# Azkellas/mesh_to_sdf

Measured on AMD Instinct MI355X. Metric: Mvoxels/s for generate_grid_sdf (512^3, 100k tris, Raycast), higher is better.
Workload: dtype f32; 1 GPU; generate_grid_sdf 512^3 grid, blob-100k (100000 tris, 50002 verts), SignMethod::Raycast, contiguous x-slabs over 1 GPU(s), whole grid resident on every GPU at the end of a step (delivery: single GPU, nothing to deliver), inputs/outputs resident in HBM; mesh=blob-100k, sign_method=Raycast, parallelism=xslab1, processes=1 (one per GPU), exchange=none, gather_chunks=1, piece_streams=1

## Files before the change

### mesh_to_sdf_amd/csrc/capi.hip

```cpp
#include <chrono>
#include <cmath>
#include <cstdarg>
#include <cstdio>
#include <cstdlib>
#include <algorithm>
#include <cstring>
#include <map>
#include <memory>
#include <mutex>
#include <thread>
#include <vector>

#include "../../include/m2s.h"
#include "capi_internal.h"
#include "common.h"
#include "sample.hip.h"
#include "tuning.h"

namespace m2s {

static thread_local char g_err[512] = "";

void set_error(const char* fmt, ...) {
  va_list ap;
// ... 2227 lines not shown
  M2S_HIP_CHECK(hipEventRecord(st->ev[2], c.stream));
  st->planes_done = nullptr;
  st->have_raw_seeds = false;
  if ((rc = remark_leaves(m, c, m->dm.leaf_max))) return rc;
  const NodeMom* moms = nullptr;
  if ((rc = mesh_winding_moments(m, c, *st, &moms))) return rc;
  if ((rc = run_grid_winding(ws, c, *st, m->dm, moms, g, slab_cells, o, d_err))) return rc;
  if (!c.sync) return park_async_events(m, *st, slab_cells, o.sdf ? 2 : 1);
  return finish_winding(c, *st, d_err, m->n_tris, slab_cells, o);
}

int m2s_cast_rays(const float* vertices, size_t n_vertices, const void* indices, size_t n_indices, int index_bytes, int topology,
                  const float* origins, const float* directions, size_t n_rays, const m2s_ray_opts* ropts, float* t_out, uint32_t* triangle_out,
                  float* uv_out, uint32_t* count_out, uint8_t* occluded_out, const m2s_opts* opts) {
  g_err[0] = 0;
  RayArgs o{t_out, triangle_out, uv_out, count_out, occluded_out, 0.0f, __builtin_inff()};
  int rc = check_mesh_args(vertices, n_vertices, indices, n_indices, index_bytes, topology);
  if (rc) return rc;
  if ((rc = check_ray_args(ropts, origins, directions, n_rays, opts, &o))) return rc;
  const size_t n_tris = m2s_triangle_count(n_vertices, n_indices, indices != nullptr, topology);
  if (!opts || opts->mem_kind == M2S_MEM_HOST) {
    if ((rc = check_host_indices(indices, n_indices, index_bytes, topology, n_vertices, n_tris))) return rc;
  }
  if (n_rays == 0) return M2S_OK;
  CallCtx c;
  DeviceState* st = nullptr;
  if ((rc = resolve_ctx(opts, &c, &st))) return rc;
  size_t need = (n_tris ? bvh_workspace_bytes(n_tris) : 0) + ray_workspace_bytes(c, n_rays) + 4096;
  if (c.mem_kind == M2S_MEM_HOST) need += align_up(n_vertices * 12) + align_up(n_indices * (size_t)(indices ? index_bytes : 0)) + 1024;
  if ((rc = ensure_capacity(*st, need))) return rc;
  Arena ws{st->base, st->cap, 0};
  int* d_err = ws.take<int>(16);
  M2S_HIP_CHECK(hipMemsetAsync(d_err, 0, 64, c.stream));
  M2S_HIP_CHECK(hipEventRecord(st->ev[0], c.stream));
  DeviceMesh mesh{};
  if (n_tris) {
    StagedMesh sm;
    if ((rc = stage_mesh(ws, c, vertices, n_vertices, indices, n_indices, index_bytes, &sm))) return rc;
    M2S_HIP_CHECK(hipEventRecord(st->ev[0], c.stream));
    rc = build_device_mesh(ws, c.stream, sm.d_verts, n_vertices, sm.d_indices, n_indices, index_bytes, topology, n_tris, d_err, &mesh,
                           nullptr, false, query_leaf_max(n_rays, n_tris, SIGN_NONE));
    if (rc) return rc;
  }
  M2S_HIP_CHECK(hipEventRecord(st->ev[1], c.stream));
  M2S_HIP_CHECK(hipEventRecord(st->ev[2], c.stream));
  st->planes_done = nullptr;
  if ((rc = run_cast_rays(ws, c, *st, mesh, origins, directions, n_rays, o))) return rc;
  return finish_call(c, *st, d_err, c.timings, n_tris, n_rays, false, true);
}

int m2s_mesh_cast_rays(m2s_mesh* m, const float* origins, const float* directions, size_t n_rays, const m2s_ray_opts* ropts, float* t_out,
                       uint32_t* triangle_out, float* uv_out, uint32_t* count_out, uint8_t* occluded_out, const m2s_opts* opts) {
  g_err[0] = 0;
  if (!m) return fail(M2S_ERR_BAD_ARG, "mesh is NULL");
  std::lock_guard<std::mutex> mlk(m->mu);
  RayArgs o{t_out, triangle_out, uv_out, count_out, occluded_out, 0.0f, __builtin_inff()};
  int rc = check_ray_args(ropts, origins, directions, n_rays, opts, &o);
  if (rc) return rc;
  m2s_opts mo;
  if ((rc = mesh_call_opts(m, opts, &mo))) return rc;
  if (n_rays == 0) return M2S_OK;
  CallCtx c;
  DeviceState* st = nullptr;
  if ((rc = resolve_ctx(&mo, &c, &st))) return rc;
  if ((rc = ensure_capacity(*st, ray_workspace_bytes(c, n_rays) + 8192))) return rc;
  Arena ws{st->base, st->cap, 0};
  int* d_err = ws.take<int>(16);
  if (c.sync) M2S_HIP_CHECK(hipMemsetAsync(d_err, 0, 64, c.stream));
  else d_err = m->d_err_async;
  if (!c.sync) reap_pending(m, false);
  M2S_HIP_CHECK(hipEventRecord(st->ev[0], c.stream));
  M2S_HIP_CHECK(hipEventRecord(st->ev[1], c.stream));
  M2S_HIP_CHECK(hipEventRecord(st->ev[2], c.stream));
  st->planes_done = nullptr;
  DeviceMesh none{};
  if (m->n_tris && (rc = remark_leaves(m, c, m->dm.leaf_max))) return rc;
  if ((rc = run_cast_rays(ws, c, *st, m->n_tris ? m->dm : none, origins, directions, n_rays, o))) return rc;
  if (!c.sync) return park_async_events(m, *st, n_rays, 1);
  return finish_call(c, *st, d_err, c.timings, m->n_tris, n_rays, false, true);
}

int m2s_sample_surface(const float* vertices, size_t n_vertices, const void* indices, size_t n_indices, int index_bytes, int topology,
                       size_t n_samples, const m2s_surface_sample_opts* sopts, float* point_out, uint32_t* triangle_out, float* uv_out,
                       float* normal_out, double* area_out, const m2s_opts* opts) {
  g_err[0] = 0;
  SampleArgs o{point_out, triangle_out, uv_out, normal_out, area_out, 0, 0};
  int rc = check_mesh_args(vertices, n_vertices, indices, n_indices, index_bytes, topology);
  if (rc) return rc;
  if ((rc = check_sample_args(sopts, n_samples, opts, &o))) return rc;
  const size_t n_tris = m2s_triangle_count(n_vertices, n_indices, indices != nullptr, topology);
  if (n_tris > ((size_t)1 << 25)) return fail(M2S_ERR_BAD_ARG, "more than 2^25 triangles");
  if (!opts || opts->mem_kind == M2S_MEM_HOST) {
    if ((rc = check_host_indices(indices, n_indices, index_bytes, topology, n_vertices, n_tris))) return rc;
  }
  if (n_tris == 0) return sample_of_nothing(o, n_samples);
  CallCtx c;
  DeviceState* st = nullptr;
  if ((rc = resolve_ctx(opts, &c, &st))) return rc;
  size_t need = sample_table_bytes(n_tris) + sample_scratch_bytes(n_tris) + sample_workspace_bytes(c, n_samples) + 4096;
  if (c.mem_kind == M2S_MEM_HOST) need += align_up(n_vertices * 12) + align_up(n_indices * (size_t)(indices ? index_bytes : 0)) + 1024;
  if ((rc = ensure_capacity(*st, need))) return rc;
  Arena ws{st->base, st->cap, 0};
  int* d_err = ws.take<int>(16);
  M2S_HIP_CHECK(hipMemsetAsync(d_err, 0, 64, c.stream));
  StagedMesh sm;
  if ((rc = stage_mesh(ws, c, vertices, n_vertices, indices, n_indices, index_bytes, &sm))) return rc;
  M2S_HIP_CHECK(hipEventRecord(st->ev[0], c.stream));
  M2S_HIP_CHECK(hipEventRecord(st->ev[1], c.stream));
  M2S_HIP_CHECK(hipEventRecord(st->ev[2], c.stream));
  st->planes_done = nullptr;
  SampleTable tb;
  if (sample_table_carve(ws, ws, n_tris, &tb)) return fail(M2S_ERR_HIP, "internal: workspace");
  const SampleSrc src{sm.d_verts, sm.d_indices, (uint32_t)n_vertices, index_bytes, topology, nullptr, nullptr, (uint32_t)n_tris};
  uint32_t amax_bits = 0;
  uint64_t W = 0;
  if ((rc = make_sample_table(c, *st, src, tb, d_err, &amax_bits, &W))) return rc;
  if (amax_bits == 0 || W == 0) return sample_of_nothing(o, n_samples);
  if (o.area) *o.area = sample_total_area(amax_bits, W);
  if ((rc = run_sample_surface(ws, c, *st, src, tb, W, n_samples, o))) return rc;
  return finish_call(c, *st, d_err, c.timings, n_tris, n_samples, false, true);
}

int m2s_mesh_sample_surface(m2s_mesh* m, size_t n_samples, const m2s_surface_sample_opts* sopts, float* point_out, uint32_t* triangle_out,
                            float* uv_out, float* normal_out, double* area_out, const m2s_opts* opts) {
  g_err[0] = 0;
  if (!m) return fail(M2S_ERR_BAD_ARG, "mesh is NULL");
  std::lock_guard<std::mutex> mlk(m->mu);
  SampleArgs o{point_out, triangle_out, uv_out, normal_out, area_out, 0, 0};
  int rc = check_sample_args(sopts, n_samples, opts, &o);
  if (rc) return rc;
  m2s_opts mo;
  if ((rc = mesh_call_opts(m, opts, &mo))) return rc;
  if (m->n_tris == 0) return sample_of_nothing(o, n_samples);
  CallCtx c;
  DeviceState* st = nullptr;
  if ((rc = resolve_ctx(&mo, &c, &st))) return rc;
  if ((rc = ensure_capacity(*st, (m->samp_mem ? 0 : sample_scratch_bytes(m->n_tris)) + sample_workspace_bytes(c, n_samples) + 8192))) return rc;
  Arena ws{st->base, st->cap, 0};
  int* d_err = ws.take<int>(16);
  if (c.sync) M2S_HIP_CHECK(hipMemsetAsync(d_err, 0, 64, c.stream));
  else d_err = m->d_err_async;
  if (!c.sync) reap_pending(m, false);
  M2S_HIP_CHECK(hipEventRecord(st->ev[0], c.stream));
  M2S_HIP_CHECK(hipEventRecord(st->ev[1], c.stream));
  M2S_HIP_CHECK(hipEventRecord(st->ev[2], c.stream));
  st->planes_done = nullptr;
  if ((rc = remark_leaves(m, c, m->dm.leaf_max))) return rc;
  const SampleSrc src{nullptr, nullptr, 0, 4, M2S_TRIANGLE_LIST, m->dm.corners, m->dm.slot_of, (uint32_t)m->n_tris};
  if (!m->samp_mem) {
    char* block = nullptr;
    const size_t bytes = sample_table_bytes(m->n_tris);
    M2S_HIP_CHECK(hipMalloc((void**)&block, bytes));
    Arena table{block, bytes, 0};
    SampleTable tb;
    rc = sample_table_carve(table, ws, m->n_tris, &tb) ? fail(M2S_ERR_HIP, "internal: workspace") : 0;
    if (!rc) rc = make_sample_table(c, *st, src, tb, nullptr, &m->samp_amax_bits, &m->samp_W);
    if (rc) { (void)hipFree(block); return rc; }
    m->samp_mem = block;
    m->samp = tb;
    m->samp.A = nullptr;
    m->samp.tile_sum = nullptr;
  }
  if (m->samp_amax_bits == 0 || m->samp_W == 0) return sample_of_nothing(o, n_samples);
  if (o.area) *o.area = sample_total_area(m->samp_amax_bits, m->samp_W);
  if ((rc = run_sample_surface(ws, c, *st, src, m->samp, m->samp_W, n_samples, o))) return rc;
  if (!c.sync) return park_async_events(m, *st, n_samples, 1);
  return finish_call(c, *st, d_err, c.timings, m->n_tris, n_samples, false, true);
}

int m2s_peer_bandwidth(const float* src, float* const* peers, uint32_t n_peers, size_t n_cells, int device, float* gbps_each, float* gbps_all) {
  g_err[0] = 0;
  if (!src || (n_peers && !peers) || n_peers > M2S_MAX_PEERS) return fail(M2S_ERR_BAD_ARG, "m2s_peer_bandwidth: bad arguments");
  if (n_cells == 0 || n_peers == 0) { if (gbps_all) *gbps_all = 0.0f; return M2S_OK; }
  int ndev = 0;
  if (hipGetDeviceCount(&ndev) != hipSuccess || ndev <= 0) return fail(M2S_ERR_HIP, "no HIP device available");
  if (device < 0) M2S_HIP_CHECK(hipGetDevice(&device));
  if (device >= ndev) return fail(M2S_ERR_BAD_ARG, "device %d out of range (%d devices)", device, ndev);
  int prev_device = device;
  (void)hipGetDevice(&prev_device);
  struct Guard {
    hipStream_t st = nullptr;
    hipEvent_t a = nullptr, b = nullptr;
    int restore;
    ~Guard() {
      if (a) (void)hipEventDestroy(a);
      if (b) (void)hipEventDestroy(b);
      if (st) (void)hipStreamDestroy(st);
      (void)hipSetDevice(restore);
    }
  } guard;
  guard.restore = prev_device;
  M2S_HIP_CHECK(hipSetDevice(device));
  M2S_HIP_CHECK(hipStreamCreateWithFlags(&guard.st, hipStreamNonBlocking));
  M2S_HIP_CHECK(hipEventCreate(&guard.a));
  M2S_HIP_CHECK(hipEventCreate(&guard.b));
  const hipStream_t st = guard.st;
  const hipEvent_t a = guard.a, b = guard.b;
  int rc = M2S_OK;
  auto timed = [&](const PeerOut& po, float* gbps) -> int {
    float best = 0.0f;
    for (int rep = 0; rep < 4; ++rep) {
      M2S_HIP_CHECK(hipEventRecord(a, st));
      const int r = launch_push_cells(st, src, po, 0, n_cells);
      if (r) return r;
      M2S_HIP_CHECK(hipEventRecord(b, st));
      M2S_HIP_CHECK(hipStreamSynchronize(st));
      float ms = 0.0f;
      M2S_HIP_CHECK(hipEventElapsedTime(&ms, a, b));
      if (rep && ms > 0.0f) best = std::max(best, (float)((double)n_cells * 4.0 * po.n / (ms * 1e-3) / 1e9));
    }
    *gbps = best;
    return 0;
  };
  for (uint32_t k = 0; k < n_peers && !rc; ++k) {
    if (!peers[k]) { rc = fail(M2S_ERR_BAD_ARG, "m2s_peer_bandwidth: peers[%u] is NULL", k); break; }
    PeerOut one{};
    one.n = 1;
    one.p[0] = peers[k];
    float g = 0.0f;
    rc = timed(one, &g);
    if (gbps_each) gbps_each[k] = g;
  }
  if (!rc && gbps_all) {
    PeerOut all{};
    all.n = n_peers;
    for (uint32_t k = 0; k < n_peers; ++k) all.p[k] = peers[k];
    rc = timed(all, gbps_all);
  }
  return rc;
}

int m2s_tuning_set(const char* name, const char* value) {
  clear_error();
  if (tuning_set(name, value) != 0) return fail(M2S_ERR_BAD_ARG, "m2s_tuning_set: unknown knob or unparsable value: %s=%s", name ? name : "(null)", value ? value : "(default)");
  return M2S_OK;
}
int m2s_tuning_describe(char* buffer, int capacity) { return tuning_describe(buffer, capacity); }

int m2s_debug_mesh_digest(m2s_mesh* m, uint64_t out[8]) {
  g_err[0] = 0;
  if (!m || !out) return fail(M2S_ERR_BAD_ARG, "NULL argument");
  std::lock_guard<std::mutex> mlk(m->mu);
  M2S_HIP_CHECK(hipSetDevice(m->device));
  M2S_HIP_CHECK(hipDeviceSynchronize());
  const size_t n = m->n_tris, nn = n ? 2 * n - 1 : 0;
  const void* ptr[7] = {m->dm.tris, m->dm.planes, m->dm.nodes, m->dm.ext, m->dm.cen, m->dm.slot_of, m->dm.scene};
  const size_t bytes[7] = {n * sizeof(TriRec), n * sizeof(TriPlanes), nn * sizeof(NodeRec), nn * sizeof(NodeExt), n * 16, n * 4, n ? 32u : 0u};
  std::vector<unsigned char> h;
  for (int k = 0; k < 7; ++k) {
    uint64_t f = 1469598103934665603ull;
    if (bytes[k]) {
      h.resize(bytes[k]);
      M2S_HIP_CHECK(hipMemcpy(h.data(), ptr[k], bytes[k], hipMemcpyDeviceToHost));
      for (size_t i = 0; i < bytes[k]; ++i) { f ^= h[i]; f *= 1099511628211ull; }
    }
    out[k] = f;
  }
  out[7] = n;
  return M2S_OK;
}

int m2s_debug_cut_code(uint32_t n_nodes, uint32_t start, uint32_t len, uint32_t out[3]) {
  g_err[0] = 0;
  if (!out || n_nodes == 0 || n_nodes > (1u << 26) || len == 0 || start >= n_nodes || len > n_nodes - start) return fail(M2S_ERR_BAD_ARG, "bad range");
  cut_word_roundtrip(n_nodes, start, len, &out[0], &out[1], &out[2]);
  return M2S_OK;
}

int m2s_debug_leaf_sizes(const m2s_grid* grid, size_t n_tris, size_t n_queries, uint32_t out[3]) {
  g_err[0] = 0;
  if (!grid || !out) return fail(M2S_ERR_BAD_ARG, "NULL argument");
  GridParams g;
  size_t slab_cells = 0;
  const int rc = fill_grid_params(grid, nullptr, &g, &slab_cells);
  if (rc) return rc;
  out[0] = grid_leaf_max(g, n_tris);
  out[1] = query_leaf_max(n_queries, n_tris, SIGN_RAYS3);
  out[2] = query_walk_is_lane(n_queries, n_tris, SIGN_RAYS3) ? 1u : 0u;
  return M2S_OK;
}

int m2s_debug_grid_walk_choice_slab(const m2s_grid* grid, const m2s_opts* opts, size_t n_tris, size_t n_nodes, uint32_t leaf_max, int algorithm, uint32_t out[8]) {
  g_err[0] = 0;
  if (!grid || !out) return fail(M2S_ERR_BAD_ARG, "NULL argument");
  GridParams g;
  size_t slab_cells = 0;
  const int rc = fill_grid_params(grid, opts, &g, &slab_cells);
  if (rc) return rc;
  const GridWalkChoice ch = choose_grid_walk(g, n_tris, n_nodes, leaf_max, false, algorithm, tuning());
  out[0] = (uint32_t)ch.path;
  out[1] = ch.seeds ? 1u : 0u;
  out[2] = (uint32_t)ch.cut_levels;
  out[3] = ch.group_waves;
  out[4] = ch.split ? 1u : 0u;
  out[5] = ch.split_forced ? 1u : 0u;
  out[6] = (uint32_t)ch.defer;
  out[7] = choose_grid_walk_for_sizing(g, n_tris).split ? 1u : 0u;
  return M2S_OK;
}
int m2s_debug_grid_walk_choice(const m2s_grid* grid, size_t n_tris, size_t n_nodes, uint32_t leaf_max, int algorithm, uint32_t out[8]) {
  return m2s_debug_grid_walk_choice_slab(grid, nullptr, n_tris, n_nodes, leaf_max, algorithm, out);
}

}
```

### mesh_to_sdf_amd/csrc/common.h

```cpp
#pragma once
#include <functional>
#include <hip/hip_runtime.h>
#include <stddef.h>
#include <stdint.h>

namespace m2s {

struct alignas(32) TriRec {
  float ax, ay, az;
  uint32_t cls;
  float bx, by, bz;
  uint32_t index;
  float cx, cy, cz;
  float pad0;
  float abx, aby, abz, nrx;
  float acx, acy, acz, nry;
  float bcx, bcy, bcz, nrz;
};
static_assert(sizeof(TriRec) == 96, "TriRec must be 96 bytes");

struct alignas(32) NodeRec {
  float mnx, mny, mnz;
  uint32_t skip;
  float mxx, mxy, mxz;
  int32_t tri;
};
static_assert(sizeof(NodeRec) == 32, "NodeRec must be 32 bytes");

struct alignas(16) NodeExt {
  float cx, cy, cz, R;
  float nx, ny, nz, mid;
  float half;
  uint32_t skip;
  int32_t tri;
  uint32_t pad;
};
constexpr uint32_t EXT_TRIVIAL_ABOVE = 2048;
static_assert(sizeof(NodeExt) == 48, "NodeExt must be 48 bytes");

struct alignas(64) TriPlanes {
  float nx, ny, nz, dn;
  float m0x, m0y, m0z, o0;
  float m1x, m1y, m1z, o1;
  float m2x, m2y, m2z, o2;
};
static_assert(sizeof(TriPlanes) == 64, "TriPlanes must be 64 bytes");

struct DeviceMesh {
  const TriRec* tris;
  const float4* corners;
  const TriPlanes* planes;
  const float4* cen;
  const float4* cen_raw;
  const uint32_t* slot_of;
  const NodeRec* nodes;
  const NodeExt* ext;
  unsigned long long* stats;
  uint32_t n_tris;
  uint32_t n_nodes;
  uint32_t leaf_max;
  const uint32_t* slot_first;
  const int* scene;
};

__device__ __forceinline__ float mesh_scale(const DeviceMesh& m) { return __int_as_float(m.scene[6]); }

struct GridParams {
  float first[3];
  float size[3];
  uint32_t n[3];
  uint32_t xb, xe;
  uint32_t nzw;
  uint64_t out_off;
  uint32_t bl[3];
  uint32_t sz_magic, sy_magic;
  uint32_t xl_cap;
  uint32_t chunk_log, period;
};
__host__ __device__ __forceinline__ uint32_t slab_x(const GridParams& g, uint32_t v) {
  return g.xb + (v >> g.chunk_log) * g.period + (v & ((1u << g.chunk_log) - 1u));
}

inline void set_super_brick_magic(GridParams& g) {
  const uint64_t nbx = (g.n[0] + (1u << g.bl[0]) - 1u) >> g.bl[0], nby = (g.n[1] + (1u << g.bl[1]) - 1u) >> g.bl[1],
                 nbz = (g.n[2] + (1u << g.bl[2]) - 1u) >> g.bl[2];
  const uint64_t sy = (nby + 7) >> 3, sz = (nbz + 7) >> 3, n_max = (nbx + 1) * sy * sz;
  const uint64_t d_max = sy > sz ? sy : sz;
  const bool safe = n_max * d_max < (1ull << 32);
  g.sz_magic = (safe && sz > 1) ? (uint32_t)(((1ull << 32) + sz - 1) / sz) : 0u;
  g.sy_magic = (safe && sy > 1) ? (uint32_t)(((1ull << 32) + sy - 1) / sy) : 0u;
}

inline void choose_brick_shape(const float size[3], uint32_t bl[3]) {
  bl[0] = bl[1] = bl[2] = 2;
  float s[3];
  for (int k = 0; k < 3; ++k) {
    s[k] = size[k] < 0 ? -size[k] : size[k];
    if (!(s[k] > 0.0f) || !(s[k] < 3.0e38f)) return;
  }
  float best = -1.0f;
  for (uint32_t a = 0; a <= 6; ++a)
    for (uint32_t b = 0; a + b <= 6; ++b) {
      const uint32_t c = 6 - a - b;
      const float e[3] = {s[0] * (float)(1u << a), s[1] * (float)(1u << b), s[2] * (float)(1u << c)};
      const float mx = e[0] > e[1] ? (e[0] > e[2] ? e[0] : e[2]) : (e[1] > e[2] ? e[1] : e[2]);
      const float mn = e[0] < e[1] ? (e[0] < e[2] ? e[0] : e[2]) : (e[1] < e[2] ? e[1] : e[2]);
      const float ratio = mx / mn;
      const bool cube = a == 2 && b == 2;
      if (best < 0.0f || ratio < best * 0.999f || (cube && ratio <= best * 1.001f)) { best = ratio; bl[0] = a; bl[1] = b; bl[2] = c; }
    }
}

constexpr uint32_t MAX_PEERS = 15;
struct PeerOut {
  float* p[MAX_PEERS];
  uint32_t n;
  uint32_t unit_log;
  uint32_t rows;
  uint32_t units;
  uint32_t* progress;
};

enum : int { ERRF_INDEX_OOB = 1, ERRF_NAN = 2, ERRF_TRAIL_TIMEOUT = 4, ERRF_BUILD_TIMEOUT = 8, ERRF_SPLIT_OVERFLOW = 16 };

enum : int {
  MODE_UNSIGNED = 0,
  MODE_NORMAL_FOLD = 1,
  MODE_NEAREST_NORMAL = 2
};
enum : int {
  SIGN_NONE = 0,
  SIGN_GRID_PLANE = 1,
  SIGN_RAYS3 = 2,
  SIGN_XRAY_ALL = 3
};

#define M2S_HIP_CHECK(expr)                                                   \
  do {                                                                        \
    hipError_t _e = (expr);                                                   \
    if (_e != hipSuccess) {                                                   \
      ::m2s::set_error("%s failed: %s (%s:%d)", #expr, hipGetErrorString(_e), __FILE__, __LINE__); \
      return M2S_ERR_HIP_INTERNAL;                                            \
    }                                                                         \
  } while (0)

constexpr int M2S_ERR_HIP_INTERNAL = -4;
void set_error(const char* fmt, ...);

struct Arena {
  char* base = nullptr;
  size_t cap = 0;
  size_t off = 0;
  template <class T>
  T* take(size_t count, size_t align = 256) {
    size_t o = (off + align - 1) / align * align;
    size_t bytes = count * sizeof(T);
    if (o + bytes > cap) return nullptr;
    off = o + bytes;
    return reinterpret_cast<T*>(base + o);
  }
};

hipError_t sort_pairs_u64(void* tmp, size_t& bytes, const uint64_t* keys_in, uint64_t* keys_out, const uint32_t* vals_in, uint32_t* vals_out, size_t n,
                          unsigned begin_bit, unsigned end_bit, hipStream_t st);
hipError_t sort_pairs_u32(void* tmp, size_t& bytes, const uint32_t* keys_in, uint32_t* keys_out, const uint32_t* vals_in, uint32_t* vals_out, size_t n,
                          unsigned begin_bit, unsigned end_bit, hipStream_t st);
hipError_t select_flagged_indices(void* tmp, size_t& bytes, const uint8_t* flags, uint32_t* out, uint32_t* count, size_t n, hipStream_t st);
void warm_bvh(hipStream_t st);
void warm_sign(hipStream_t st);
void warm_distance(hipStream_t st);
void warm_seeds(hipStream_t st);
void warm_cut(hipStream_t st);
void warm_brute(hipStream_t st);
void warm_query_order(hipStream_t st);
void warm_peer_push(hipStream_t st);
void warm_serde(hipStream_t st);
void warm_client(hipStream_t st);
void warm_sortlib(hipStream_t st);
void warm_sortlib_query(hipStream_t st);
void warm_grid_query(hipStream_t st);
void warm_rays(hipStream_t st);
void warm_sample(hipStream_t st);
size_t bvh_workspace_bytes(size_t n_tris);
int build_device_mesh(Arena& ws, hipStream_t st, const float* d_verts, size_t n_verts, const void* d_indices,
                      size_t n_indices, int index_bytes, int topology, size_t n_tris, int* d_err, DeviceMesh* out,
                      const std::function<int(const float4*, const TriRec*, int)>* after_setup = nullptr, bool records_only = false,
                      uint32_t leaf_max = 2, uint64_t job_cells = ~0ull);
bool query_walk_is_lane(size_t n_q, size_t n_tris, int sign_src);
uint32_t query_leaf_max(size_t n_q, size_t n_tris, int sign_src);
uint32_t grid_leaf_max(const GridParams& g, size_t n_tris);
int set_leaf_size(hipStream_t st, DeviceMesh* mesh, uint32_t leaf_max);

size_t sign_workspace_bytes(const GridParams& g, size_t n_tris);
int build_grid_sign_plane(Arena& ws, hipStream_t st, const DeviceMesh& mesh, const GridParams& g,
                          const uint32_t** d_inside_plane, bool slab_only);

size_t grid_distance_workspace_bytes(const GridParams& g, size_t n_tris);
constexpr uint32_t SPLIT_MAX_ROUNDS = 6, SPLIT_CNT_WORDS = 16 + 16 * (SPLIT_MAX_ROUNDS + 1);
struct SplitCtl {
  uint32_t* cnt = nullptr;
  uint32_t* slot_packet = nullptr;
  uint32_t* acc = nullptr;
  uint4* items = nullptr;
  uint32_t cap_slots = 0, cap_items = 0;
  uint32_t grace = 0;
  uint32_t patience_q8 = 0;
  uint32_t idle_below = 0;
  uint32_t emit_min = 0, emit_max = 0;
  uint32_t rounds = 3;
};
struct Tuning;
struct GridWalkChoice {
  enum Path { NOTHING, ALL_PAIRS_SPLIT , ALL_PAIRS , LANE, GROUP, PACKET };
  Path path = NOTHING;
  bool seeds = false;
  int cut_levels = 0;
  uint32_t group_waves = 0;
  bool split = false;
  bool split_forced = false;
  int defer = 0;
};
GridWalkChoice choose_grid_walk(const GridParams& g, size_t n_tris, size_t n_nodes, uint32_t leaf_max, bool counting, int algorithm, const Tuning& tn);
GridWalkChoice choose_grid_walk_for_sizing(const GridParams& g, size_t n_tris);
struct GridWalkPlan {
  GridWalkChoice choice;
  const uint32_t* seeds = nullptr;
  uint32_t seed_shift = 0, seed_ny = 0, seed_nz = 0;
  const uint32_t* cut_lists = nullptr;
  uint32_t cut_log = 0, cut_ny = 0, cut_nz = 0;
  SplitCtl split;
  const uint2* group_top = nullptr;
  uint32_t* brute_acc = nullptr;
};
bool grid_is_tiny(const GridParams& g, size_t n_tris, int algorithm, bool raycast);
bool grid_is_tiny(const GridParams& g, size_t n_tris, int algorithm, bool raycast, const Tuning& tn);
struct SeedLattice {
  uint32_t* ids = nullptr;
  uint32_t ny = 0, nz = 0;
  size_t points = 0;
  uint32_t shift = 0;
};
bool grid_walk_wants_seeds(const GridParams& g, size_t n_tris, int algorithm);
uint32_t host_packet_bricks(const GridParams& g);
int launch_grid_seeds(Arena& ws, hipStream_t st, const float4* cen, uint32_t n_tris, const GridParams& g, SeedLattice* out);
void launch_seed_remap(hipStream_t st, uint32_t* ids, size_t n, const uint32_t* slot_of, uint32_t n_tris);
void launch_grid_cut(hipStream_t st, const DeviceMesh& mesh, const GridParams& g, const uint32_t* seeds, uint32_t seed_shift, uint32_t seed_ny,
                     uint32_t seed_nz, uint32_t* lists, uint32_t* coarse);
void launch_query_cut(hipStream_t st, const DeviceMesh& mesh, const uint32_t* seeds, uint32_t launched, uint32_t* lists, const float4* centres,
                      const uint32_t* table, const GridParams* d_lat);
int launch_grid_brute_split(hipStream_t st, const DeviceMesh& mesh, const GridParams& g, int mode, const uint32_t* plane, uint32_t* acc, uint32_t real,
                            float* d_out, int* d_err, const PeerOut& peers);
int launch_grid_brute(hipStream_t st, const DeviceMesh& mesh, const GridParams& g, int mode, const uint32_t* plane, float* d_out, int* d_err,
                      uint32_t packets, const PeerOut& peers);
int launch_query_brute(hipStream_t st, const DeviceMesh& mesh, const float* d_queries, uint32_t n_q, int mode, int sign_src, float* d_out, int* d_err);
int prepare_grid_walk(Arena& ws, hipStream_t st, const DeviceMesh& mesh, const GridParams& g, int algorithm, bool pipelined,
                      GridWalkPlan* plan, const SeedLattice* raw_seeds = nullptr);
int launch_grid_walk(hipStream_t st, const DeviceMesh& mesh, const GridParams& g, int mode, const uint32_t* d_inside_plane,
                     const GridWalkPlan& plan, uint32_t bx_off, float* d_out, int* d_err, const PeerOut* peers = nullptr);
int launch_push_cells(hipStream_t st, const float* src, const PeerOut& peers, uint64_t first, uint64_t count);
uint32_t trail_unit_log(const GridParams& g);
uint32_t trail_units(const GridParams& g);
uint32_t trail_rows(const GridParams& g);
int launch_push_trailing(hipStream_t st, const float* src, const PeerOut& peers, const GridParams& g, int* d_err);
int launch_grid_distance(Arena& ws, hipStream_t st, const DeviceMesh& mesh, const GridParams& g, int mode,
                         const uint32_t* d_inside_plane, int algorithm, float* d_out, int* d_err,
                         hipEvent_t ev_before_final, hipEvent_t wait_before_final = nullptr, bool pipelined = false,
                         const SeedLattice* raw_seeds = nullptr, hipEvent_t wait_raw_seeds = nullptr,
                         const PeerOut* peers = nullptr);
void cut_word_roundtrip(uint32_t n_nodes, uint32_t start, uint32_t len, uint32_t* word, uint32_t* first, uint32_t* end);
size_t query_workspace_bytes(size_t n_q);
bool query_is_tiny(size_t n_q, size_t n_tris, int algorithm, int sign_src);
int launch_query_brute_split(Arena& ws, hipStream_t st, const DeviceMesh& mesh, const float* d_queries, size_t n_q, int mode, int sign_src,
                             float* d_out, int* d_err);
struct QueryPlan {
  size_t n_q = 0;
  const int* qb = nullptr;
  const uint32_t* perm = nullptr;
  const float4* sorted = nullptr;
  const uint32_t* table = nullptr;
  const float4* centres = nullptr;
  const GridParams* lat = nullptr;
  uint32_t launched = 0;
  bool lane_walk = false, seeds = false;
};
struct QuerySeeds {
  uint32_t* ids = nullptr;
  bool raw = false;
};
int prepare_query_walk(Arena& ws, hipStream_t st, const float* d_queries, size_t n_q, size_t n_tris, int sign_src, int algorithm, QueryPlan* plan,
                       hipEvent_t after_lattice = nullptr);
int launch_query_seeds(Arena& ws, hipStream_t st, const float4* cen, uint32_t n_tris, const QueryPlan& plan, bool raw, QuerySeeds* out);
int launch_query_walk(Arena& ws, hipStream_t st, const DeviceMesh& mesh, const float* d_queries, const QueryPlan& plan,
                      int mode, int sign_src, int algorithm, float* d_out, int* d_err, const QuerySeeds* pre = nullptr);
int launch_query_distance(Arena& ws, hipStream_t st, const DeviceMesh& mesh, const float* d_queries, size_t n_q,
                          int mode, int sign_src, int algorithm, float* d_out, int* d_err);

struct ClosestOut {
  uint32_t* tri;
  float* point;
  float* dist;
  uint64_t off;
};
int launch_closest_grid(hipStream_t st, const DeviceMesh& mesh, const GridParams& g, const float* d_dist, uint64_t dist_off, int algorithm,
                        const ClosestOut& out);
int launch_closest_queries(hipStream_t st, const DeviceMesh& mesh, const float* d_queries, const uint32_t* perm, size_t n_q, const float* d_dist,
                           int algorithm, const ClosestOut& out);

struct alignas(64) NodeMom {
  float cx, cy, cz;
  float r;
  float ax, ay, az;
  float m[9];
};
static_assert(sizeof(NodeMom) == 64, "NodeMom must be 64 bytes");
struct WindingOut {
  float* w;
  float* sdf;
  uint64_t off;
};
int launch_winding_moments(hipStream_t st, const DeviceMesh& mesh, NodeMom* moms);
int launch_winding_grid(hipStream_t st, const DeviceMesh& mesh, const NodeMom* moms, const GridParams& g, float beta, float threshold,
                        const float* d_dist, uint64_t dist_off, int algorithm, const WindingOut& out);
int launch_winding_queries(hipStream_t st, const DeviceMesh& mesh, const NodeMom* moms, const float* d_queries, const uint32_t* perm, size_t n_q,
                           float beta, float threshold, const float* d_dist, int algorithm, const WindingOut& out);


struct RayOut {
  float* t;
  uint32_t* tri;
  float* uv;
  uint32_t* count;
  uint8_t* occluded;
};
int launch_cast_rays(hipStream_t st, const DeviceMesh& mesh, const float* d_org, const float* d_dir, size_t n_rays, float t_min, float t_max,
                     int algorithm, const RayOut& out);

struct SampleSrc {
  const float* verts;
  const void* indices;
  uint32_t n_verts;
  int index_bytes, topology;
  const float4* corners;
  const uint32_t* slot_of;
  uint32_t n_tris;
};
constexpr uint32_t SAMPLE_TOP = 2048;
struct SampleTable {
  uint64_t* C;
  uint64_t* top;
  uint32_t* hdr;
  float* A;
  uint64_t* tile_sum;
};
struct SampleOut {
  float* point;
  uint32_t* tri;
  float* uv;
  float* normal;
};
size_t sample_table_bytes(size_t n_tris);
size_t sample_scratch_bytes(size_t n_tris);
int sample_table_carve(Arena& table, Arena& scratch, size_t n_tris, SampleTable* tb);
int launch_sample_table(hipStream_t st, const SampleSrc& src, const SampleTable& tb, int* d_err);
int launch_sample_surface(hipStream_t st, const SampleSrc& src, const SampleTable& tb, uint64_t W, uint64_t seed, uint64_t first, size_t n_samples,
                          int algorithm, const SampleOut& out);

struct GridQuery {
  float start[3], end[3], cs[3];
  int64_t n[3];
  uint64_t nyz;
  float iso, outside;
  float eps;
  uint32_t max_steps;
};
int launch_sample_grid(hipStream_t st, const GridQuery& q, int mode, const float* d, const float* pts, uint64_t n, float* value_out,
                       float* normal_out);
int launch_raymarch_grid(hipStream_t st, const GridQuery& q, int mode, const float* d, const float* org, const float* dir, uint64_t n,
                         float* hit_out, uint32_t* steps_out, float* normal_out);


struct wire_bytes { uint8_t b[120]; uint32_t n; };
int launch_write_bytes(hipStream_t st, uint8_t* d_dst, const uint8_t* bytes, uint32_t n);
int launch_encode_f32(hipStream_t st, const float* d_values, uint64_t n, uint8_t* d_dst);
int launch_encode_points(hipStream_t st, const float* d_points, uint64_t n, uint8_t* d_dst);
int launch_decode_f32(hipStream_t st, const uint8_t* d_src, uint64_t n, float* d_out, int* d_err);
int launch_decode_points(hipStream_t st, const uint8_t* d_src, uint64_t n, float* d_out, int* d_err);

size_t order_workspace_bytes(size_t n);
int launch_order_cells(Arena& ws, hipStream_t st, const float* d_dist, size_t n, uint32_t* d_ordered, float* d_limits);
struct InstanceDev {
  const void* vertices;
  const uint32_t* indices;
  uint64_t stride;
  float m[16];
};
size_t merge_workspace_bytes();
int launch_merge_instances(Arena& ws, hipStream_t st, const InstanceDev* d_inst, const uint64_t* d_vfirst, const uint64_t* d_ifirst,
                           uint32_t n_inst, uint64_t n_vertices, uint64_t n_indices, float* d_vertices, uint32_t* d_indices,
                           float* d_bbox);

}
```

### mesh_to_sdf_amd/csrc/dist.hip.h

```cpp
#pragma once
#include "common.h"
#include "walk.hip.h"

namespace m2s {

namespace {

#ifndef M2S_CUT_MAX
#define M2S_CUT_MAX 15
#endif
__host__ __device__ __forceinline__ uint32_t cut_start_bits(uint32_t n_nodes) {
  uint32_t b = 1;
  while (b < 27u && (1u << b) < n_nodes) ++b;
  return b;
}
__host__ __device__ __forceinline__ uint32_t cut_decode_len(uint32_t code, uint32_t M) { return (code & ((1u << M) - 1u)) << (code >> M); }
__host__ __device__ __forceinline__ uint32_t cut_encode_len(uint32_t len, uint32_t M) {
  if (len < (1u << M)) return len;
  uint32_t e = (32u - (uint32_t)__builtin_clz(len)) - M;
  uint32_t mant = (len + (1u << e) - 1u) >> e;
  if (mant == (1u << M)) { mant >>= 1; ++e; }
  return (e << M) | mant;
}
constexpr uint32_t CUT_MAX = M2S_CUT_MAX, CUT_WORDS = M2S_CUT_MAX + 1;
static_assert(M2S_CUT_MAX <= 15, "the range count has four bits");
struct CutList {
  const uint32_t* lists;
  uint32_t log, ny, nz;
  uint32_t bx_off;
  const float4* centres;
};
constexpr uint32_t CUTC_S_LOG = 3, CUTC_S = 1u << CUTC_S_LOG, CUTC_WORDS = 8, CUTC_MAX = CUTC_WORDS - 1;
static_assert(CUTC_S * CUTC_WORDS == 64, "a fine wave fetches its block's coarse record with one load, lane = word");

__device__ __forceinline__ bool query_packet_range(const uint32_t* __restrict__ table, uint32_t packet, uint32_t n_q,
                                                   uint32_t* first, uint32_t* cnt) {
  uint32_t f = packet * 64u, c = 64u;
  if (table != nullptr) {
    const uint32_t count = table[0];
    if (packet >= count) return false;
    if (table[1] == 0u) {
      f = table[2u + packet];
      c = (packet + 1u < count ? table[3u + packet] : n_q) - f;
    }
  }
  if (f >= n_q) return false;
  *first = f;
  *cnt = min(c, n_q - f);
  return true;
}
__device__ __forceinline__ uint32_t query_lattice_cell(const GridParams& L, float x, float y, float z) {
  const float q0[3] = {x, y, z};
  uint32_t cell[3];
  for (int k = 0; k < 3; ++k) {
    float f = (q0[k] - L.first[k]) / L.size[k] + 0.5f;
    f = (f == f) ? fminf(fmaxf(f, 0.0f), (float)(L.n[k] - 1)) : 0.0f;
    cell[k] = min((uint32_t)f, L.n[k] - 1);
  }
  return (cell[0] * L.n[1] + cell[1]) * L.n[2] + cell[2];
}
constexpr uint32_t QL = 64;

template <int M, int S>
struct WalkForm { static constexpr int MODE = M, SIGN = S; };
template <class F>
void for_grid_form(int mode, bool planes, F&& f) {
  if (mode == MODE_UNSIGNED && planes) f(WalkForm<MODE_UNSIGNED, SIGN_GRID_PLANE>{});
  else if (mode == MODE_UNSIGNED) f(WalkForm<MODE_UNSIGNED, SIGN_NONE>{});
  else f(WalkForm<MODE_NORMAL_FOLD, SIGN_NONE>{});
}
template <class F>
void for_query_form(int mode, int sign_src, F&& f) {
  if (mode == MODE_UNSIGNED && sign_src == SIGN_RAYS3) f(WalkForm<MODE_UNSIGNED, SIGN_RAYS3>{});
  else if (mode == MODE_UNSIGNED) f(WalkForm<MODE_UNSIGNED, SIGN_NONE>{});
  else if (mode == MODE_NORMAL_FOLD) f(WalkForm<MODE_NORMAL_FOLD, SIGN_NONE>{});
  else f(WalkForm<MODE_NEAREST_NORMAL, SIGN_NONE>{});
}

struct BrickCounts { uint32_t nb[3]; uint64_t real, grid; uint32_t padded; };
static bool slab_is_empty(const GridParams& g) { return g.xe <= g.xb || g.n[1] == 0 || g.n[2] == 0; }
BrickCounts brick_counts(const GridParams& g) {
  BrickCounts c;
  c.nb[0] = bricks_along(g.xe - g.xb, g.bl[0]), c.nb[1] = bricks_along(g.n[1], g.bl[1]), c.nb[2] = bricks_along(g.n[2], g.bl[2]);
  c.real = (uint64_t)c.nb[0] * c.nb[1] * c.nb[2];
  c.grid = (uint64_t)bricks_along(g.n[0], g.bl[0]) * c.nb[1] * c.nb[2];
  const uint32_t xl = super_brick_xlog(c.nb[0], g.xl_cap);
  c.padded = ((c.nb[0] + (1u << xl) - 1u) >> xl) * ((c.nb[1] + 7) >> 3) * ((c.nb[2] + 7) >> 3) * (64u << xl);
  return c;
}
static size_t cut_blocks(const GridParams& g, uint32_t log) {
  const BrickCounts bc = brick_counts(g);
  return (size_t)bricks_along(bc.nb[0], log) * bricks_along(bc.nb[1], log) * bricks_along(bc.nb[2], log);
}

}

}
```

### mesh_to_sdf_amd/csrc/distance.hip

```cpp
#include <algorithm>
#include <cmath>
#include <cstdio>
#include <cstdlib>
#include <cstring>
#include <type_traits>

#include "common.h"
#include "geo.hip.h"
#include "tuning.h"
#include "walk.hip.h"
#include "dist.hip.h"

namespace m2s {

namespace {

template <int AXIS>
__device__ __forceinline__ uint32_t stab_count(const DeviceMesh& mesh, f3 p) {
  uint32_t count = 0;
  uint32_t node = 0;
  while (node < mesh.n_nodes) {
    node = __builtin_amdgcn_readfirstlane(node);
    const NodeRec nr = record_at(mesh.nodes, node);
    const bool hit = ray_meets_box<AXIS>(p, mk3(nr.mnx, nr.mny, nr.mnz), mk3(nr.mxx, nr.mxy, nr.mxz));
// ... 91 lines not shown
__device__ __forceinline__ uint32_t split_peek(const uint32_t* addr) {
  uint32_t v;
  const uint32_t zero = 0;
  asm volatile("s_nop 4\n\tglobal_load_dword %0, %1, %2 nt\n\ts_waitcnt vmcnt(0)" : "=v"(v) : "v"(zero), "s"(addr));
  return (uint32_t)__builtin_amdgcn_readfirstlane((int)v);
}
__device__ __forceinline__ void split_poke(uint32_t* addr, uint32_t value) {
  const uint32_t zero = 0;
  asm volatile("s_nop 4\n\tglobal_store_dword %0, %1, %2" : : "v"(zero), "v"(value), "s"(addr));
}
__device__ __forceinline__ uint32_t split_now() { return (uint32_t)__builtin_amdgcn_s_memrealtime(); }
__device__ __forceinline__ void split_arm(SplitState& sp, const SplitCtl& ctl, uint32_t round, bool may_suspend) {
  if (ctl.cnt == nullptr || !may_suspend) return;
  sp.flag_addr = split_flag_addr(ctl, round);
  sp.next_check = ctl.grace;
  sp.grace = ctl.grace;
  sp.patience_q8 = ctl.patience_q8;
}
__device__ __forceinline__ bool split_stragglers_only(const SplitState& sp) {
  const uint32_t up = split_peek(sp.flag_addr);
  if (up == 0u) return false;
  const uint32_t start = split_peek(sp.flag_addr + 8), now = split_now();
  const uint32_t fill = up - start;
  const uint32_t allowed = (uint32_t)(((unsigned long long)fill * sp.patience_q8) >> 8);
  return now - up >= allowed;
}

template <int MODE>
__device__ __forceinline__ bool split_handover(const SplitCtl& split, uint32_t packet, uint32_t range, uint32_t off, const Best<MODE>& best, int* err) {
  const uint32_t lane = threadIdx.x & 63u;
  uint32_t slot = 0, idx = 0;
  if (lane == 0u) slot = atomicAdd(&split.cnt[0], 1u);
  slot = __builtin_amdgcn_readfirstlane(slot);
  if (slot >= split.cap_slots) return false;
  if (lane == 0u) idx = atomicAdd(&split.cnt[2], 1u);
  idx = __builtin_amdgcn_readfirstlane(idx);
  if (idx >= split.cap_items) {
    if (lane == 0u) split.slot_packet[slot] = 0xffffffffu;
    return false;
  }
  constexpr uint32_t AW = MODE == MODE_NORMAL_FOLD ? 128u : 64u;
  uint32_t* acc = split.acc + (size_t)slot * AW;
  acc[lane] = __float_as_uint(best.d2);
  if (MODE == MODE_NORMAL_FOLD) {
    acc[64 + lane] = __float_as_uint(best.d2pos);
    if (best.nan) atomicOr(err, ERRF_NAN);
  }
  if (lane == 0u) {
    split.items[idx] = make_uint4(packet, off, range, slot | SPLIT_CONTINUATION);
    split.slot_packet[slot] = packet;
  }
  return true;
}

struct EmitState {
  uint4* list = nullptr;
  uint32_t* count = nullptr;
  uint32_t cap = 0;
  uint32_t base = 0, used = 0, room = 0;
  uint32_t min_bytes = 0xffffffffu, max_bytes = 0;
  uint32_t packet = 0, slot = 0;
};
__device__ __forceinline__ void emit_begin(EmitState& em, const SplitCtl& ctl, uint32_t next_round, uint32_t packet, uint32_t slot) {
  em.list = ctl.items + (size_t)(next_round - 1u) * ctl.cap_items;
  em.count = ctl.cnt + 1u + next_round;
  em.cap = ctl.cap_items;
  em.min_bytes = ctl.emit_min;
  em.max_bytes = ctl.emit_max;
  em.packet = packet;
  em.slot = slot;
}
__device__ __forceinline__ void emit_close(EmitState& em) {
  const uint32_t i = em.base + em.used + (threadIdx.x & 63u);
  if (i < em.base + em.room && i < em.cap) em.list[i] = make_uint4(em.packet, 0u, 0u, em.slot);
  em.used = em.room;
}
__device__ __forceinline__ void emit_reserve(EmitState& em) {
  uint32_t base = 0;
  if ((threadIdx.x & 63u) == 0u) base = atomicAdd(em.count, 64u);
  em.base = __builtin_amdgcn_readfirstlane(base);
  em.used = 0;
  em.room = 64u;
  if (em.base + 64u > em.cap) {
    emit_close(em);
    em.room = 0;
    em.min_bytes = 0xffffffffu;
  }
}

template <int MODE>
struct DeferLayout {
  static constexpr uint32_t SLOT_WORDS = MODE == MODE_NORMAL_FOLD ? 192u : MODE == MODE_NEAREST_NORMAL ? 128u : 64u;
  static constexpr uint32_t DWORDS = (256u + SLOT_WORDS) / 2u;
};
constexpr uint32_t DEFER_DIRECT_LANES = 48;
struct DeferQueue {
  uint32_t* q;
  uint32_t* slot;
  uint32_t head, n;
  uint32_t* q1;
  uint32_t head1, n1;
};
__device__ __forceinline__ void wave_lds_sync() {
  __builtin_amdgcn_fence(__ATOMIC_RELEASE, "wavefront");
  __builtin_amdgcn_wave_barrier();
  __builtin_amdgcn_fence(__ATOMIC_ACQUIRE, "wavefront");
}
template <int MODE>
__device__ __forceinline__ unsigned long long defer_key(const Best<MODE>& x) {
  return ((unsigned long long)__float_as_uint(x.d2) << 32) | ((unsigned long long)(x.idx & 0x7fffffffu) << 1) | (x.pos ? 0ull : 1ull);
}
template <int MODE>
__device__ __forceinline__ DeferQueue defer_begin(unsigned long long* lds) {
  const uint32_t lane = threadIdx.x & 63u;
  DeferQueue dq = {reinterpret_cast<uint32_t*>(lds), reinterpret_cast<uint32_t*>(lds) + 256, 0u, 0u, reinterpret_cast<uint32_t*>(lds) + 128, 0u, 0u};
  if (MODE == MODE_NEAREST_NORMAL) reinterpret_cast<unsigned long long*>(dq.slot)[lane] = 0x7f800000ffffffffull;
  else {
    dq.slot[lane] = 0x7f800000u;
    if (MODE == MODE_NORMAL_FOLD) { dq.slot[64u + lane] = 0x7f800000u; dq.slot[128u + lane] = 0u; }
  }
  return dq;
}
template <int MODE>
__device__ __forceinline__ void defer_flush(const DeviceMesh& mesh, f3 p, DeferQueue& dq, Best<MODE>& best) {
  const uint32_t lane = threadIdx.x & 63u;
  wave_lds_sync();
  const uint32_t take = min(dq.n, 64u);
  const bool valid = lane < take;
  const uint32_t e = valid ? dq.q[(dq.head + lane) & 127u] : 0u;
  const uint32_t v = e & 63u, t = e >> 6;
  const f3 pv = mk3(__shfl(p.x, (int)v), __shfl(p.y, (int)v), __shfl(p.z, (int)v));
  Best<MODE> one;
  eval_triangle<MODE>(one, pv, mesh.tris[t]);
  if (valid) {
    if (MODE == MODE_NEAREST_NORMAL) atomicMin(&reinterpret_cast<unsigned long long*>(dq.slot)[v], defer_key<MODE>(one));
    else {
      atomicMin(&dq.slot[v], __float_as_uint(one.d2));
      if (MODE == MODE_NORMAL_FOLD) {
        atomicMin(&dq.slot[64u + v], __float_as_uint(one.d2pos));
        if (one.nan) dq.slot[128u + v] = 1u;
      }
    }
  }
  dq.head = (dq.head + take) & 127u;
  dq.n -= take;
  wave_lds_sync();
  if (MODE == MODE_NEAREST_NORMAL) {
    const unsigned long long kk = reinterpret_cast<const unsigned long long*>(dq.slot)[lane];
    if (kk < defer_key<MODE>(best)) { best.d2 = __uint_as_float((uint32_t)(kk >> 32)); best.idx = (uint32_t)(kk >> 1) & 0x7fffffffu; best.pos = (kk & 1ull) == 0ull; }
  } else {
    best.d2 = fminf(best.d2, __uint_as_float(dq.slot[lane]));
    if (MODE == MODE_NORMAL_FOLD) { best.d2pos = fminf(best.d2pos, __uint_as_float(dq.slot[64u + lane])); best.nan |= dq.slot[128u + lane] != 0u; }
  }
}
template <int MODE>
__device__ __forceinline__ bool defer_pretest(const DeviceMesh& mesh, f3 p, float thr, DeferQueue& dq, Best<MODE>& best) {
  const uint32_t lane = threadIdx.x & 63u;
  wave_lds_sync();
  const uint32_t take = min(dq.n1, 64u);
  const bool valid = lane < take;
  const uint32_t e = valid ? dq.q1[(dq.head1 + lane) & 127u] : 0u;
  const uint32_t v = e & 63u, t = e >> 6;
  const f3 pv = mk3(__shfl(p.x, (int)v), __shfl(p.y, (int)v), __shfl(p.z, (int)v));
  const float tv = __shfl(thr, (int)v);
  const bool pass = valid & !(planes_dist2(pv, mesh.planes[t]) > tv);
  dq.head1 = (dq.head1 + take) & 127u;
  dq.n1 -= take;
  const unsigned long long rb = __ballot(pass);
  if (rb == 0ull) return false;
  const uint32_t rank = __builtin_amdgcn_mbcnt_hi((uint32_t)(rb >> 32), __builtin_amdgcn_mbcnt_lo((uint32_t)rb, 0u));
  if (pass) dq.q[(dq.head + dq.n + rank) & 127u] = e;
  dq.n += (uint32_t)__popcll(rb);
  if (dq.n < 64u) return false;
  defer_flush<MODE>(mesh, p, dq, best);
  return true;
}
template <int MODE>
__device__ __forceinline__ void defer_drain(const DeviceMesh& mesh, f3 p, float slack, DeferQueue& dq, Best<MODE>& best) {
  while (dq.n1 != 0u) defer_pretest<MODE>(mesh, p, prune_bound(best.d2, slack), dq, best);
  while (dq.n != 0u) defer_flush<MODE>(mesh, p, dq, best);
}

template <int MODE, bool STATS, bool BUDGET, bool EMIT = false, bool HANDOVER = false, int DEFER = 0>
__device__ __forceinline__ void walk_span(const DeviceMesh& mesh, f3 p, float slack, Best<MODE>& best, float& thr, uint32_t& off,
                                          uint32_t end, WalkStats& st, SplitState& sp, EmitState* emp = nullptr, DeferQueue* dqp = nullptr) {
  constexpr uint32_t NB = (uint32_t)sizeof(NodeExt);
  while (off < end) {
    off = __builtin_amdgcn_readfirstlane(off);
    const NodeExt nr = record_at_bytes<NodeExt>(mesh.ext, off);
    if (STATS) ++st.box;
    const float ed2 = ext_dist2(p, nr);
    if (STATS) st.node_lanes += (uint32_t)__popcll(__ballot(!(ed2 > thr)));
    if (STATS && __ballot(!(ed2 > thr)) == 0ull) {
      ++st.pruned;
      const float vx = p.x - nr.cx, vy = p.y - nr.cy, vz = p.z - nr.cz;
      const float t = nr.nz * vz + nr.ny * vy + nr.nx * vx, sl = fmaxf(fabsf(t - nr.mid) - nr.half, 0.0f);
      if (__ballot(!(sl * sl > thr)) == 0ull) ++st.slab;
      const float rs = __builtin_amdgcn_sqrtf(nr.R * nr.R + (fabsf(nr.mid) + nr.half) * (fabsf(nr.mid) + nr.half));
      const float sq = fmaxf(__builtin_amdgcn_sqrtf(vx * vx + vy * vy + vz * vz) - rs, 0.0f);
      if (__ballot(!(sq * sq > thr)) == 0ull) ++st.sphere;
    }
    if (__ballot(!(ed2 > thr)) == 0ull) { off = nr.skip; continue; }
    if (nr.tri >= 0) {
      const uint32_t cnt = (nr.skip - off + NB) / (2u * NB);
      if (DEFER == 3) {
        DeferQueue& dq = *dqp;
        const bool want = !(ed2 > thr);
        const unsigned long long wb = __ballot(want);
        const uint32_t rank = __builtin_amdgcn_mbcnt_hi((uint32_t)(wb >> 32), __builtin_amdgcn_mbcnt_lo((uint32_t)wb, 0u));
        const uint32_t wn = (uint32_t)__popcll(wb);
        for (uint32_t k = 0; k < cnt; ++k) {
          if (want) dq.q1[(dq.head1 + dq.n1 + rank) & 127u] = (threadIdx.x & 63u) | (((uint32_t)nr.tri + k) << 6);
          dq.n1 += wn;
          if (dq.n1 >= 64u) {
            if (BUDGET) sp.units += 4u;
            if (defer_pretest<MODE>(mesh, p, thr, dq, best)) thr = prune_bound(best.d2, slack);
          }
        }
      } else
      for (uint32_t k = 0; k < cnt; ++k) {
        if (STATS) { ++st.ext; st.pre_lanes += (uint32_t)__popcll(__ballot(!(ed2 > thr))); }
        const TriPlanes tp = record_at(mesh.planes, (uint32_t)nr.tri + k);
        const bool reach = !(planes_dist2(p, tp) > thr);
        const unsigned long long rb = __ballot(reach);
        if (rb != 0ull) {
          if (STATS) { ++st.leaf; st.pairs += (uint32_t)__popcll(rb); }
          if (DEFER != 0 && !(DEFER == 2 && (uint32_t)__popcll(rb) >= DEFER_DIRECT_LANES)) {
            DeferQueue& dq = *dqp;
            const uint32_t rank = __builtin_amdgcn_mbcnt_hi((uint32_t)(rb >> 32), __builtin_amdgcn_mbcnt_lo((uint32_t)rb, 0u));
            if (reach) dq.q[(dq.head + dq.n + rank) & 127u] = (threadIdx.x & 63u) | (((uint32_t)nr.tri + k) << 6);
            dq.n += (uint32_t)__popcll(rb);
            if (dq.n >= 64u) {
              if (BUDGET) sp.units += 4u;
              defer_flush<MODE>(mesh, p, dq, best);
              thr = prune_bound(best.d2, slack);
            }
          } else {
            if (BUDGET) sp.units += 4u;
            const TriRec tr = record_at_vec(mesh.tris, (uint32_t)nr.tri + k);
            eval_triangle_leaf<MODE>(best, p, tr, reach);
            thr = prune_bound(best.d2, slack);
          }
        }
      }
      off = nr.skip;
      if (BUDGET) {
        sp.units += 3u + cnt;
        if (sp.units >= sp.next_check) {
          bool go;
          if (HANDOVER) go = split_stragglers_only(sp);
          else {
            go = sp.flag_seen;
            if (!go && split_peek(sp.flag_addr) != 0u) { sp.flag_seen = true; sp.next_check = sp.units + sp.grace; }
          }
          if (go) {
            if (off < end || HANDOVER) { sp.suspended = true; sp.resume_end = end; end = off; if (HANDOVER) *sp.n_ranges = 0u; }
            sp.next_check = 0xffffffffu;
          } else if (HANDOVER || !sp.flag_seen) {
            sp.next_check = sp.units + SPLIT_CHECK_EVERY;
          }
        }
      }
    } else {
      if (EMIT) {
        EmitState& em = *emp;
        const uint32_t bytes = nr.skip - off;
        if (bytes >= em.min_bytes && bytes <= em.max_bytes) {
          if (em.used == em.room) emit_reserve(em);
          if (em.used < em.room) {
            if ((threadIdx.x & 63u) == 0u) em.list[em.base + em.used] = make_uint4(em.packet, off, nr.skip, em.slot);
            ++em.used;
            off = nr.skip;
            continue;
          }
        }
      }
      off = off + NB;
    }
  }
}

__device__ __forceinline__ void store_grid_result(float* __restrict__ out, size_t out_index, float result, bool store, const GridParams& g,
                                                  const GridBrick& vox, const PeerOut& peers, int lane) {
  if (peers.progress != nullptr) {
    if (store) __hip_atomic_store(&out[out_index], result, __ATOMIC_RELAXED, __HIP_MEMORY_SCOPE_AGENT);
    asm volatile("s_waitcnt vmcnt(0)" ::: "memory");
    if (lane == 0) {
      const uint32_t unit = vox.bx >> peers.unit_log;
      const uint32_t nbx = bricks_along(g.xe - g.xb, g.bl[0]), nbz = bricks_along(g.n[2], g.bl[2]);
      const uint32_t bricks = min((unit + 1u) << peers.unit_log, nbx) - (unit << peers.unit_log);
      const uint32_t old = __hip_atomic_fetch_add(&peers.progress[peers.units + unit * peers.rows + vox.by], 1u, __ATOMIC_RELAXED, __HIP_MEMORY_SCOPE_AGENT);
      if (old + 1u == bricks * nbz) __hip_atomic_fetch_add(&peers.progress[unit], 1u, __ATOMIC_RELAXED, __HIP_MEMORY_SCOPE_AGENT);
    }
    return;
  }
  if (store) out[out_index] = result;
  if (peers.n != 0u && store) {
    const size_t gi = out_index + (size_t)g.out_off;
    for (uint32_t i = 0; i < peers.n; ++i) peers.p[i][gi] = result;
  }
}

template <bool GRID, int MODE, int SIGN, bool STATS, bool SPLIT, int DEFER = 0>
__global__ __launch_bounds__(64) __attribute__((amdgpu_waves_per_eu(8, 8))) void k_packet(DeviceMesh mesh, GridParams g, const float4* __restrict__ qsorted,
                                               const uint32_t* __restrict__ perm, uint32_t n_q,
                                               const uint32_t* __restrict__ plane, float* __restrict__ out,
                                               int* __restrict__ err, uint32_t n_packets,
                                               const uint32_t* __restrict__ seed_in, uint32_t seed_shift,
                                               uint32_t seed_ny, uint32_t seed_nz,
                                               const GridParams* __restrict__ seed_lattice, CutList cut, PeerOut peers, SplitCtl split) {
  const int lane = threadIdx.x & 63;
  if (SPLIT && (blockIdx.x < 8u || blockIdx.x + 8u >= gridDim.x) && lane == 0) {
    const uint32_t t = split.idle_below  ? 0u : split_now();
    if (blockIdx.x < 8u) split_poke(split_flag_addr(split, 0u) + 8, t);
    if (blockIdx.x + 8u >= gridDim.x) split_poke(split_flag_addr(split, 0u), t | 1u);
  }
  const uint32_t block = xcd_remap(blockIdx.x);
  const uint32_t packet = (uint32_t)__builtin_amdgcn_readfirstlane((int)block);
  if (packet >= n_packets) return;

  f3 p;
  size_t out_index;
  bool store;
  GridBrick vox{};
  if (GRID) {
    vox = grid_lane_voxel(g, packet, lane);
    if (!vox.brick_in_grid) return;
    p = grid_point(g, vox);
    out_index = ((size_t)vox.x * g.n[1] + vox.y) * g.n[2] + vox.z - (size_t)g.out_off;
    store = vox.in_range;
  } else {
    uint32_t first, cnt;
    if (!query_packet_range(plane, packet, n_q, &first, &cnt)) return;
    const uint32_t i = first + min((uint32_t)lane, cnt - 1u);
    const float4 q = qsorted[i];
    p = mk3(q.x, q.y, q.z);
    out_index = perm[i];
    store = (uint32_t)lane < cnt;
  }

  Best<MODE> best;
  WalkStats st;
  uint32_t st_ranges = 0, st_band = 0, st_rbytes = 0;
  if (mesh.n_nodes) {
    const float scale = fmaxf(mesh_scale(mesh), fmaxf(fabsf(p.x), fmaxf(fabsf(p.y), fabsf(p.z))));
    const float slack = 4.0e-6f * scale + (MODE == MODE_NORMAL_FOLD ? 2.5e-6f : 0.0f);
    SplitState sp;
    if (SPLIT) split_arm(sp, split, 0u, true);
    __shared__ unsigned long long defer_lds[DEFER ? DeferLayout<MODE>::DWORDS : 1];
    DeferQueue dq = {nullptr, nullptr, 0u, 0u};
    if (DEFER) dq = defer_begin<MODE>(defer_lds);

    constexpr uint32_t NB = (uint32_t)sizeof(NodeExt);
    const uint32_t* cl = nullptr;
    uint32_t n_ranges = 1, cut_off_v = 0, cut_end_v = (lane == 1) ? mesh.n_nodes * NB : 0u;
    if (SPLIT) sp.n_ranges = &n_ranges;
    if (cut.lists != nullptr) {
      const uint32_t cb = GRID ? __builtin_amdgcn_readfirstlane((((vox.bx + cut.bx_off) >> cut.log) * cut.ny + (vox.by >> cut.log)) * cut.nz + (vox.bz >> cut.log))
                               : packet;
      cl = cut.lists + (size_t)cb * CUT_WORDS;
      const uint32_t cw = cl[(uint32_t)lane & 15u];
      const uint32_t cS = cut_start_bits(mesh.n_nodes), cfirst = cw & ((1u << cS) - 1u);
      const uint32_t clen = ((cw >> cS) & ((1u << (27u - cS)) - 1u)) << (cw >> 27);
      cut_off_v = cfirst * NB;
      cut_end_v = min(cfirst + clen, mesh.n_nodes) * NB;
      n_ranges = __builtin_amdgcn_readfirstlane(cw);
    }
    if (seed_in != nullptr) {
      uint32_t sidx = packet;
      if (GRID) {
        sidx = (((vox.bx + cut.bx_off) >> seed_shift) * seed_ny + (vox.by >> seed_shift)) * seed_nz + (vox.bz >> seed_shift);
      } else {
        const GridParams L = *seed_lattice;
        float q0[3] = {__shfl(p.x, 0), __shfl(p.y, 0), __shfl(p.z, 0)};
        if (cut.centres != nullptr) {
          const float4 c = cut.centres[packet];
          q0[0] = c.x; q0[1] = c.y; q0[2] = c.z;
        }
        sidx = __builtin_amdgcn_readfirstlane(query_lattice_cell(L, q0[0], q0[1], q0[2]));
      }
      const uint32_t slot = __builtin_amdgcn_readfirstlane(min(seed_in[sidx], mesh.n_tris - 1));
      const TriRec tr = record_at(mesh.tris, slot);
      eval_triangle<MODE>(best, p, tr);
    } else {
      const f3 c = {__shfl(p.x, 0), __shfl(p.y, 0), __shfl(p.z, 0)};
      uint32_t n = 0;
      NodeRec nr = mesh.nodes[0];
      while (nr.tri < 0) {
        const uint32_t l = n + 1;
        const NodeRec nl = mesh.nodes[l];
        const uint32_t r = nl.skip;
        const NodeRec nrr = mesh.nodes[r];
        const float dl = box_dist2(c, nl.mnx, nl.mny, nl.mnz, nl.mxx, nl.mxy, nl.mxz);
        const float dr = box_dist2(c, nrr.mnx, nrr.mny, nrr.mnz, nrr.mxx, nrr.mxy, nrr.mxz);
        const bool go_left = __builtin_amdgcn_readfirstlane((int)(dl <= dr)) != 0;
        n = go_left ? l : r;
        nr = go_left ? nl : nrr;
      }
      const TriRec tr = mesh.tris[nr.tri];
      eval_triangle<MODE>(best, p, tr);
    }

    float thr = prune_bound(best.d2, slack);
    if (STATS && GRID) {
      const float cells = __shfl(__builtin_amdgcn_sqrtf(best.d2), 0) / fabsf(g.size[0]);
      st_band = cells < 1.0f ? 0u : min(7u, 1u + (uint32_t)__builtin_amdgcn_readfirstlane((int)floorf(log2f(cells))));
      st_band = __builtin_amdgcn_readfirstlane(st_band);
    }
    const int passes = (STATS && mesh.stats != nullptr && mesh.stats[7] == 2ull) ? 2 : 1;
    for (int pass = 0; pass < passes; ++pass) {
      if (pass == 1) { st.box = 0; st.ext = 0; st.leaf = 0; }
      if (STATS) st_ranges = n_ranges;
      uint32_t range = 0, off = 0;
      for (; range < n_ranges; ++range) {
        off = (uint32_t)__builtin_amdgcn_readlane((int)cut_off_v, (int)(1u + range));
        const uint32_t end = (uint32_t)__builtin_amdgcn_readlane((int)cut_end_v, (int)(1u + range));
        if (STATS) st_rbytes += end - off;
        walk_span<MODE, STATS, SPLIT, false, SPLIT, DEFER>(mesh, p, slack, best, thr, off, end, st, sp, nullptr, &dq);
      }
      if (DEFER) defer_drain<MODE>(mesh, p, slack, dq, best);
      if (SPLIT && sp.suspended) {
        if (!split_handover<MODE>(split, packet, range - 1u, off, best, err)) atomicOr(err, ERRF_SPLIT_OVERFLOW);
        return;
      }
    }
  }

  if (STATS && mesh.stats != nullptr && lane == 0) {
    atomicAdd(&mesh.stats[0], (unsigned long long)st.box);
    atomicAdd(&mesh.stats[1], (unsigned long long)st.ext);
    atomicAdd(&mesh.stats[2], (unsigned long long)st.leaf);
    atomicAdd(&mesh.stats[3], 1ull);
    atomicAdd(&mesh.stats[4], (unsigned long long)st.pruned);
    atomicAdd(&mesh.stats[5], (unsigned long long)st.slab);
    atomicAdd(&mesh.stats[6], (unsigned long long)st.sphere);
    atomicMax(&mesh.stats[72], (unsigned long long)st.box);
    atomicMax(&mesh.stats[73], (unsigned long long)st.leaf);
    atomicMax(&mesh.stats[74], (unsigned long long)(st.box + st.ext + 4u * st.leaf));
    atomicAdd(&mesh.stats[75], (unsigned long long)st.node_lanes);
    atomicAdd(&mesh.stats[76], (unsigned long long)st.pre_lanes);
    atomicAdd(&mesh.stats[77], (unsigned long long)st.pairs);
    unsigned long long* q = mesh.stats + 8 + 8 * st_band;
    atomicAdd(&q[0], (unsigned long long)st.box);
    atomicAdd(&q[1], (unsigned long long)st.ext);
    atomicAdd(&q[2], (unsigned long long)st.leaf);
    atomicAdd(&q[3], 1ull);
    atomicAdd(&q[4], (unsigned long long)st_ranges);
    atomicAdd(&q[5], (unsigned long long)st.pairs);
    atomicAdd(&q[6], (unsigned long long)st_rbytes);
    atomicAdd(&q[7], (unsigned long long)(st_rbytes <= 4096u ? 1u : 0u));
    const uint32_t units = st.box + st.ext + 4u * st.leaf;
    atomicAdd(&mesh.stats[80 + (31 - __builtin_clz(units | 1u))], 1ull);
  }

  bool negate = false;
  if (MODE == MODE_UNSIGNED) {
    if (SIGN == SIGN_GRID_PLANE) {
      const size_t w = ((size_t)vox.x * g.n[1] + vox.y) * g.nzw + (vox.z >> 5);
      negate = (plane[w] >> (vox.z & 31u)) & 1u;
    } else if (SIGN == SIGN_RAYS3) {
      __shared__ uint32_t ray_lds[DEFER != 0 ? 192 : 1];
      const uint32_t cx = DEFER != 0 ? stab_count_dense<0>(mesh, p, ray_lds) : stab_count<0>(mesh, p);
      const uint32_t cy = DEFER != 0 ? stab_count_dense<1>(mesh, p, ray_lds) : stab_count<1>(mesh, p);
      uint32_t cz = cx;
      if (__ballot(((cx ^ cy) & 1u) != 0u) != 0ull) cz = DEFER != 0 ? stab_count_dense<2>(mesh, p, ray_lds) : stab_count<2>(mesh, p);
      negate = ((cx & 1u) + (cy & 1u) + (cz & 1u)) > 1u;
    }
  }
  if (MODE == MODE_NORMAL_FOLD && best.nan) atomicOr(err, ERRF_NAN);
  const float result = finish<MODE>(best, negate);
  if (GRID) store_grid_result(out, out_index, result, store, g, vox, peers, lane);
  else if (store) out[out_index] = result;
}

constexpr uint32_t GROUP_MAX_WAVES = 4, TOP_LOG = 8, TOP_SUBTREES = 1u << TOP_LOG;
__global__ __launch_bounds__(TOP_SUBTREES) void k_tree_top(DeviceMesh mesh, uint2* __restrict__ top) {
  constexpr uint32_t NB = (uint32_t)sizeof(NodeExt);
  const uint32_t sub = threadIdx.x;
  uint32_t off = 0, end = mesh.n_nodes * NB;
  for (uint32_t lv = 0; lv < TOP_LOG && off < end; ++lv) {
    const NodeExt* nr = reinterpret_cast<const NodeExt*>(reinterpret_cast<const char*>(mesh.ext) + off);
    const uint32_t rest = sub & ((1u << (TOP_LOG - lv)) - 1u);
    if (nr->tri >= 0) { if (rest != 0u) end = off; break; }
    const uint32_t skip = nr->skip, left = off + NB;
    const uint32_t right = reinterpret_cast<const NodeExt*>(reinterpret_cast<const char*>(mesh.ext) + left)->skip;
    if ((sub >> (TOP_LOG - 1u - lv)) & 1u) { off = right; end = skip; } else { off = left; end = right; }
  }
  top[sub] = make_uint2(off, end);
}
template <int MODE, int SIGN>
__global__ __launch_bounds__(64 * GROUP_MAX_WAVES) __attribute__((amdgpu_waves_per_eu(8, 8))) void k_packet_group(
    DeviceMesh mesh, GridParams g, const uint32_t* __restrict__ plane, float* __restrict__ out, int* __restrict__ err, uint32_t n_packets,
    const uint32_t* __restrict__ seed_in, uint32_t seed_shift, uint32_t seed_ny, uint32_t seed_nz, uint32_t bx_off, const uint2* __restrict__ top, PeerOut peers) {
  static_assert(MODE == MODE_UNSIGNED || MODE == MODE_NORMAL_FOLD, "grid modes");
  const int lane = threadIdx.x & 63;
  const uint32_t wave = (uint32_t)__builtin_amdgcn_readfirstlane((int)(threadIdx.x >> 6));
  const uint32_t packet = (uint32_t)__builtin_amdgcn_readfirstlane((int)xcd_remap(blockIdx.x));
  if (packet >= n_packets) return;
  const GridBrick vox = grid_lane_voxel(g, packet, lane);
  if (!vox.brick_in_grid) return;
  const f3 p = grid_point(g, vox);
  const size_t out_index = ((size_t)vox.x * g.n[1] + vox.y) * g.n[2] + vox.z - (size_t)g.out_off;

  extern __shared__ unsigned long long group_lds[];
  const uint32_t GROUP_WAVES = blockDim.x >> 6;
  uint32_t* const lds = reinterpret_cast<uint32_t*>(group_lds);
  DeferQueue dq = {lds + wave * 256u, lds + GROUP_WAVES * 256u, 0u, 0u, lds + wave * 256u + 128u, 0u, 0u};
  if (wave == 0u) {
    dq.slot[lane] = 0x7f800000u;
    if (MODE == MODE_NORMAL_FOLD) { dq.slot[64 + lane] = 0x7f800000u; dq.slot[128 + lane] = 0u; }
  }
  Best<MODE> best;
  if (mesh.n_nodes) {
    const float scale = fmaxf(mesh_scale(mesh), fmaxf(fabsf(p.x), fmaxf(fabsf(p.y), fabsf(p.z))));
    const float slack = 4.0e-6f * scale + (MODE == MODE_NORMAL_FOLD ? 2.5e-6f : 0.0f);
    uint32_t slot = 0;
    if (seed_in != nullptr) {
      const uint32_t sidx = (((vox.bx + bx_off) >> seed_shift) * seed_ny + (vox.by >> seed_shift)) * seed_nz + (vox.bz >> seed_shift);
      slot = __builtin_amdgcn_readfirstlane(min(seed_in[sidx], mesh.n_tris - 1));
    }
    eval_triangle<MODE>(best, p, record_at(mesh.tris, slot));
    float thr = prune_bound(best.d2, slack);
    __syncthreads();
    WalkStats st;
    SplitState sp;
    for (uint32_t k = wave; k < TOP_SUBTREES; k += GROUP_WAVES) {
      const uint2 r = top[k];
      uint32_t off = (uint32_t)__builtin_amdgcn_readfirstlane((int)r.x);
      const uint32_t end = (uint32_t)__builtin_amdgcn_readfirstlane((int)r.y);
      if (off >= end) continue;
      walk_span<MODE, false, false, false, false, 3>(mesh, p, slack, best, thr, off, end, st, sp, nullptr, &dq);
    }
    defer_drain<MODE>(mesh, p, slack, dq, best);
    atomicMin(&dq.slot[lane], __float_as_uint(best.d2));
    if (MODE == MODE_NORMAL_FOLD) {
      atomicMin(&dq.slot[64 + lane], __float_as_uint(best.d2pos));
      if (best.nan) dq.slot[128 + lane] = 1u;
    }
    __syncthreads();
    if (wave != 0u) return;
    best.d2 = __uint_as_float(dq.slot[lane]);
    if (MODE == MODE_NORMAL_FOLD) { best.d2pos = __uint_as_float(dq.slot[64 + lane]); best.nan = dq.slot[128 + lane] != 0u; }
  } else if (wave != 0u) return;

  bool negate = false;
  if (MODE == MODE_UNSIGNED && SIGN == SIGN_GRID_PLANE) {
    const size_t w = ((size_t)vox.x * g.n[1] + vox.y) * g.nzw + (vox.z >> 5);
    negate = (plane[w] >> (vox.z & 31u)) & 1u;
  }
  if (MODE == MODE_NORMAL_FOLD && best.nan) atomicOr(err, ERRF_NAN);
  store_grid_result(out, out_index, finish<MODE>(best, negate), vox.in_range, g, vox, peers, lane);
}

template <int MODE>
__global__ __launch_bounds__(64) __attribute__((amdgpu_waves_per_eu(8, 8))) void k_split_round(DeviceMesh mesh, GridParams g, SplitCtl split, CutList cut, uint32_t round, bool final, int* __restrict__ err) {
  constexpr uint32_t AW = MODE == MODE_NORMAL_FOLD ? 128u : 64u;
  constexpr uint32_t NB = (uint32_t)sizeof(NodeExt);
  const int lane = threadIdx.x & 63;
  const uint32_t n_items = min(split.cnt[1u + round], split.cap_items);
  const uint4* list = split.items + (size_t)(round - 1u) * split.cap_items;
  for (uint32_t i = blockIdx.x; i < n_items; i += gridDim.x) {
    const uint4 it = list[i];
    const uint32_t packet = __builtin_amdgcn_readfirstlane(it.x), third = __builtin_amdgcn_readfirstlane(it.z), tag = __builtin_amdgcn_readfirstlane(it.w);
    const uint32_t slot = tag & ~SPLIT_CONTINUATION;
    const bool continuation = (tag & SPLIT_CONTINUATION) != 0u;
    uint32_t off = __builtin_amdgcn_readfirstlane(it.y);
    if (!continuation && off >= third) continue;
    const GridBrick vox = grid_lane_voxel(g, packet, lane);
    const f3 p = grid_point(g, vox);
    const float scale = fmaxf(mesh_scale(mesh), fmaxf(fabsf(p.x), fmaxf(fabsf(p.y), fabsf(p.z))));
    const float slack = 4.0e-6f * scale + (MODE == MODE_NORMAL_FOLD ? 2.5e-6f : 0.0f);
    uint32_t* acc = split.acc + (size_t)slot * AW;
    Best<MODE> best;
    const uint32_t d2_in = acc[lane];
    uint32_t d2pos_in = 0x7f800000u;
    best.d2 = __uint_as_float(d2_in);
    if (MODE == MODE_NORMAL_FOLD) { d2pos_in = acc[64 + lane]; best.d2pos = __uint_as_float(d2pos_in); }
    float thr = prune_bound(best.d2, slack);
    WalkStats st;
    SplitState idle;
    EmitState em;
    __shared__ unsigned long long defer_lds[DeferLayout<MODE>::DWORDS];
    wave_lds_sync();
    DeferQueue dq = defer_begin<MODE>(defer_lds);
    if (continuation) {
      uint32_t n_ranges = 1, cut_off_v = 0, cut_end_v = (lane == 1) ? mesh.n_nodes * NB : 0u;
      if (cut.lists != nullptr) {
        const uint32_t cb = __builtin_amdgcn_readfirstlane((((vox.bx + cut.bx_off) >> cut.log) * cut.ny + (vox.by >> cut.log)) * cut.nz + (vox.bz >> cut.log));
        const uint32_t cw = cut.lists[(size_t)cb * CUT_WORDS + ((uint32_t)lane & 15u)];
        const uint32_t cS = cut_start_bits(mesh.n_nodes), cfirst = cw & ((1u << cS) - 1u);
        const uint32_t clen = ((cw >> cS) & ((1u << (27u - cS)) - 1u)) << (cw >> 27);
        cut_off_v = cfirst * NB;
        cut_end_v = min(cfirst + clen, mesh.n_nodes) * NB;
        n_ranges = __builtin_amdgcn_readfirstlane(cw);
      }
      if (!final) emit_begin(em, split, round + 1u, packet, slot);
      for (uint32_t range = third; range < n_ranges; ++range) {
        if (range != third) off = (uint32_t)__builtin_amdgcn_readlane((int)cut_off_v, (int)(1u + range));
        const uint32_t end = (uint32_t)__builtin_amdgcn_readlane((int)cut_end_v, (int)(1u + range));
        walk_span<MODE, false, false, true, false, 3>(mesh, p, slack, best, thr, off, end, st, idle, &em, &dq);
      }
      emit_close(em);
    } else {
      SplitState sp;
      split_arm(sp, split, round, !final);
      walk_span<MODE, false, true, false, false, 3>(mesh, p, slack, best, thr, off, third, st, sp, nullptr, &dq);
      if (sp.suspended) {
        emit_begin(em, split, round + 1u, packet, slot);
        walk_span<MODE, false, false, true, false, 3>(mesh, p, slack, best, thr, off, sp.resume_end, st, idle, &em, &dq);
        emit_close(em);
      }
    }
    defer_drain<MODE>(mesh, p, slack, dq, best);
    if (__float_as_uint(best.d2) < d2_in) atomicMin(&acc[lane], __float_as_uint(best.d2));
    if (MODE == MODE_NORMAL_FOLD) {
      if (__float_as_uint(best.d2pos) < d2pos_in) atomicMin(&acc[64 + lane], __float_as_uint(best.d2pos));
      if (best.nan) atomicOr(err, ERRF_NAN);
    }
  }
  if (!final && lane == 0) split_poke(split_flag_addr(split, round), 1u);
}

template <int MODE, int SIGN>
__global__ __launch_bounds__(256) void k_split_finish(GridParams g, const uint32_t* __restrict__ plane, float* __restrict__ out, SplitCtl split, PeerOut peers) {
  constexpr uint32_t AW = MODE == MODE_NORMAL_FOLD ? 128u : 64u;
  const int lane = threadIdx.x & 63;
  const uint32_t n_slots = min(split.cnt[0], split.cap_slots);
  for (uint32_t slot = blockIdx.x * 4u + (threadIdx.x >> 6); slot < n_slots; slot += gridDim.x * 4u) {
    const uint32_t packet = split.slot_packet[slot];
    if (packet == 0xffffffffu) continue;
    const GridBrick vox = grid_lane_voxel(g, packet, lane);
    const uint32_t* acc = split.acc + (size_t)slot * AW;
    Best<MODE> best;
    best.d2 = __uint_as_float(acc[lane]);
    if (MODE == MODE_NORMAL_FOLD) best.d2pos = __uint_as_float(acc[64 + lane]);
    bool negate = false;
    if (MODE == MODE_UNSIGNED && SIGN == SIGN_GRID_PLANE) {
      const size_t w = ((size_t)vox.x * g.n[1] + vox.y) * g.nzw + (vox.z >> 5);
      negate = (plane[w] >> (vox.z & 31u)) & 1u;
    }
    const float result = finish<MODE>(best, negate);
    const size_t out_index = ((size_t)vox.x * g.n[1] + vox.y) * g.n[2] + vox.z - (size_t)g.out_off;
    store_grid_result(out, out_index, result, vox.in_range, g, vox, peers, lane);
  }
}
__global__ void k_split_init(uint32_t* __restrict__ cnt, uint32_t forced) {
  for (uint32_t i = threadIdx.x; i < SPLIT_CNT_WORDS; i += blockDim.x) cnt[i] = i >= 16u ? forced : 0u;
}

#ifndef M2S_LANE_WAVES
#define M2S_LANE_WAVES 6
#endif
template <int MODE>
__device__ __forceinline__ void walk_range(const DeviceMesh& mesh, f3 p, float slack, Best<MODE>& best, float& thr, uint32_t& off,
                                           uint32_t limit, uint32_t max_steps, uint32_t& st_nodes, uint32_t& st_exact) {
  constexpr uint32_t NB = (uint32_t)sizeof(NodeExt);
  const char* ext_bytes = reinterpret_cast<const char*>(mesh.ext);
  for (uint32_t s = 0; s < max_steps && off < limit; ++s) {
    const NodeExt nr = *reinterpret_cast<const NodeExt*>(ext_bytes + off);
    ++st_nodes;
    if (ext_dist2(p, nr) > thr) { off = nr.skip; continue; }
    if (nr.tri >= 0) {
      const uint32_t cnt = (nr.skip - off + NB) / (2u * NB);
      for (uint32_t k = 0; k < cnt; ++k) {
        if (!(planes_dist2(p, mesh.planes[nr.tri + k]) > thr)) {
          eval_triangle<MODE>(best, p, mesh.tris[nr.tri + k]);
          thr = prune_bound(best.d2, slack);
          ++st_exact;
        }
      }
      off = nr.skip;
    } else {
      off += NB;
    }
  }
}
struct LaneShare {
  unsigned long long key[64];
  uint32_t a[64], b[64];
  uint32_t flag[64];
  uint32_t rng[64][3];
  float4 pt[64];
};
template <int MODE>
__device__ __forceinline__ void lane_tree_walk(const DeviceMesh& mesh, f3 p, float slack, Best<MODE>& best, bool valid,
                                               uint32_t& st_nodes, uint32_t& st_exact, LaneShare& sh) {
  constexpr uint32_t NB = (uint32_t)sizeof(NodeExt);
  constexpr uint32_t ROUND = 64;
  const uint32_t end = mesh.n_nodes * NB;
  const uint32_t lane = threadIdx.x & 63u;
  auto key_of = [](const Best<MODE>& x) {
    return ((unsigned long long)__float_as_uint(x.d2) << 32) | ((unsigned long long)(x.idx & 0x7fffffffu) << 1) | (x.pos ? 0ull : 1ull);
  };
  sh.pt[lane] = make_float4(p.x, p.y, p.z, slack);
  sh.a[lane] = __float_as_uint(best.d2);
  sh.b[lane] = __float_as_uint(best.d2pos);
  sh.flag[lane] = best.nan ? 1u : 0u;
  if (MODE == MODE_NEAREST_NORMAL) sh.key[lane] = key_of(best);
  uint32_t owner = lane, off = valid ? 0u : end, limit = end;
  f3 tp = p;
  float tsl = slack;
  Best<MODE> b = best;
  float thr = prune_bound(b.d2, tsl);
  for (;;) {
    walk_range<MODE>(mesh, tp, tsl, b, thr, off, limit, ROUND, st_nodes, st_exact);
    const unsigned long long unf = __ballot(off < limit);
    if (unf == ~0ull) continue;
    if (MODE == MODE_NEAREST_NORMAL) atomicMin(&sh.key[owner], key_of(b));
    else {
      atomicMin(&sh.a[owner], __float_as_uint(b.d2));
      if (MODE == MODE_NORMAL_FOLD) { atomicMin(&sh.b[owner], __float_as_uint(b.d2pos)); if (b.nan) atomicOr(&sh.flag[owner], 1u); }
    }
    if (unf == 0ull) break;
    const uint32_t K = (uint32_t)__popcll(unf);
    if (off < limit) {
      const uint32_t r = (uint32_t)__popcll(unf & ((1ull << lane) - 1ull));
      sh.rng[r][0] = off; sh.rng[r][1] = limit; sh.rng[r][2] = owner;
    }
    __builtin_amdgcn_fence(__ATOMIC_RELEASE, "wavefront");
    __builtin_amdgcn_wave_barrier();
    __builtin_amdgcn_fence(__ATOMIC_ACQUIRE, "wavefront");
    const uint32_t k = lane % K, idx = lane / K, helpers = (64u - k + K - 1u) / K;
    const uint32_t so = sh.rng[k][0], se = sh.rng[k][1], sowner = sh.rng[k][2];
    const uint32_t records = (se - so) / NB, piece = (records + helpers - 1u) / helpers;
    off = min(se, so + idx * piece * NB);
    limit = min(se, off + piece * NB);
    owner = sowner;
    const float4 q = sh.pt[owner];
    tp = mk3(q.x, q.y, q.z);
    tsl = q.w;
    b = Best<MODE>();
    if (MODE == MODE_NEAREST_NORMAL) {
      const unsigned long long kk = sh.key[owner];
      b.d2 = __uint_as_float((uint32_t)(kk >> 32)); b.idx = (uint32_t)(kk >> 1) & 0x7fffffffu; b.pos = (kk & 1ull) == 0ull;
      if (b.idx == 0x7fffffffu) b.idx = 0xffffffffu;
    } else {
      b.d2 = __uint_as_float(sh.a[owner]);
      if (MODE == MODE_NORMAL_FOLD) b.d2pos = __uint_as_float(sh.b[owner]);
    }
    thr = prune_bound(b.d2, tsl);
    __builtin_amdgcn_fence(__ATOMIC_RELEASE, "wavefront");
    __builtin_amdgcn_wave_barrier();
    __builtin_amdgcn_fence(__ATOMIC_ACQUIRE, "wavefront");
  }
  __builtin_amdgcn_fence(__ATOMIC_RELEASE, "wavefront");
  __builtin_amdgcn_wave_barrier();
  __builtin_amdgcn_fence(__ATOMIC_ACQUIRE, "wavefront");
  if (MODE == MODE_NEAREST_NORMAL) {
    const unsigned long long kk = sh.key[lane];
    best.d2 = __uint_as_float((uint32_t)(kk >> 32)); best.idx = (uint32_t)(kk >> 1) & 0x7fffffffu; best.pos = (kk & 1ull) == 0ull;
  } else {
    best.d2 = __uint_as_float(sh.a[lane]);
    if (MODE == MODE_NORMAL_FOLD) { best.d2pos = __uint_as_float(sh.b[lane]); best.nan = sh.flag[lane] != 0u; }
  }
}

template <int MODE>
__device__ __forceinline__ void greedy_leaf(const DeviceMesh& mesh, f3 p, Best<MODE>& best) {
  uint32_t n = 0;
  NodeRec nr = mesh.nodes[0];
  while (nr.tri < 0) {
    const uint32_t l = n + 1;
    const NodeRec nl = mesh.nodes[l];
    const uint32_t r = nl.skip;
    const NodeRec nrr = mesh.nodes[r];
    const float dl = box_dist2(p, nl.mnx, nl.mny, nl.mnz, nl.mxx, nl.mxy, nl.mxz);
    const float dr = box_dist2(p, nrr.mnx, nrr.mny, nrr.mnz, nrr.mxx, nrr.mxy, nrr.mxz);
    const bool go_left = dl <= dr;
    n = go_left ? l : r;
    nr = go_left ? nl : nrr;
  }
  const uint32_t cnt = (nr.skip - n + 1u) >> 1;
  for (uint32_t k = 0; k < cnt; ++k) eval_triangle<MODE>(best, p, mesh.tris[(uint32_t)nr.tri + k]);
}

template <int MODE, int SIGN>
__global__ __launch_bounds__(256) __attribute__((amdgpu_waves_per_eu(M2S_LANE_WAVES, 8))) void k_lane(DeviceMesh mesh, GridParams g, const uint32_t* __restrict__ plane,
                                              float* __restrict__ out, int* __restrict__ err, uint32_t n_packets,
                                              const uint32_t* __restrict__ seed_in, uint32_t seed_shift, uint32_t seed_ny, uint32_t seed_nz,
                                              uint32_t bx_off, PeerOut peers) {
  const int lane = threadIdx.x & 63;
  const uint32_t packet = blockIdx.x * (blockDim.x >> 6) + (threadIdx.x >> 6);
  if (packet >= n_packets) return;
  const GridBrick vox = grid_lane_voxel(g, packet, lane);
  if (!vox.brick_in_grid) return;
  const f3 p = grid_point(g, vox);
  const size_t out_index = ((size_t)vox.x * g.n[1] + vox.y) * g.n[2] + vox.z - (size_t)g.out_off;
  const bool LANE_VALID = vox.in_range;

  Best<MODE> best;
  if (mesh.n_nodes) {
    const float scale = fmaxf(mesh_scale(mesh), fmaxf(fabsf(p.x), fmaxf(fabsf(p.y), fabsf(p.z))));
    const float slack = 4.0e-6f * scale + (MODE == MODE_NORMAL_FOLD ? 2.5e-6f : 0.0f);
    uint32_t slot = 0;
    if (seed_in != nullptr)
      slot = min(seed_in[(((vox.bx + bx_off) >> seed_shift) * seed_ny + (vox.by >> seed_shift)) * seed_nz + (vox.bz >> seed_shift)], mesh.n_tris - 1);
    eval_triangle<MODE>(best, p, mesh.tris[slot]);
    greedy_leaf<MODE>(mesh, p, best);
    uint32_t st_nodes = 0, st_exact = 0;
    __shared__ LaneShare lane_share[4];
    lane_tree_walk<MODE>(mesh, p, slack, best, LANE_VALID, st_nodes, st_exact, lane_share[threadIdx.x >> 6]);
    if (mesh.stats != nullptr && LANE_VALID) {
      atomicAdd(&mesh.stats[0], (unsigned long long)st_nodes);
      atomicAdd(&mesh.stats[2], (unsigned long long)st_exact);
      atomicAdd(&mesh.stats[3], 1ull);
      atomicMax(&mesh.stats[72], (unsigned long long)st_nodes);
      atomicMax(&mesh.stats[73], (unsigned long long)st_exact);
    }
  }
  bool negate = false;
  if (MODE == MODE_UNSIGNED && SIGN == SIGN_GRID_PLANE) {
    const size_t w = ((size_t)vox.x * g.n[1] + vox.y) * g.nzw + (vox.z >> 5);
    negate = (plane[w] >> (vox.z & 31u)) & 1u;
  }
  if (MODE == MODE_NORMAL_FOLD && best.nan) atomicOr(err, ERRF_NAN);
  const float result = finish<MODE>(best, negate);
  if (vox.in_range) {
    out[out_index] = result;
    for (uint32_t i = 0; i < peers.n; ++i) peers.p[i][out_index + (size_t)g.out_off] = result;
  }
}

template <int AXIS>
__device__ __forceinline__ uint32_t stab_count_lane(const DeviceMesh& mesh, f3 p) {
  uint32_t count = 0, node = 0;
  while (node < mesh.n_nodes) {
    const NodeRec nr = mesh.nodes[node];
    if (!ray_meets_box<AXIS>(p, mk3(nr.mnx, nr.mny, nr.mnz), mk3(nr.mxx, nr.mxy, nr.mxz))) { node = nr.skip; continue; }
    if (nr.tri >= 0) {
      const uint32_t cnt = (nr.skip - node + 1u) >> 1;
      for (uint32_t k = 0; k < cnt; ++k) {
        const uint32_t vi = 3u * ((uint32_t)nr.tri + k);
        const float4 c0 = mesh.corners[vi], c1 = mesh.corners[vi + 1u], c2 = mesh.corners[vi + 2u];
        const f3 a = mk3(c0.x, c0.y, c0.z), b = mk3(c0.w, c1.x, c1.y), c = mk3(c1.z, c1.w, c2.x);
        f3 mn, mx;
        triangle_bounding_box(a, b, c, &mn, &mx);
        float t;
        const bool h = ray_meets_box<AXIS>(p, mn, mx) && ray_triangle_aligned<AXIS>(p, a, b, c, &t);
        count += h ? 1u : 0u;
      }
      node = nr.skip;
    } else {
      node = node + 1;
    }
  }
  return count;
}
template <int MODE, int SIGN>
__global__ __launch_bounds__(256) __attribute__((amdgpu_waves_per_eu(M2S_LANE_WAVES, 8))) void k_lane_q(DeviceMesh mesh, const float4* __restrict__ qsorted, const uint32_t* __restrict__ perm,
                                                uint32_t n_q, float* __restrict__ out, int* __restrict__ err,
                                                const uint32_t* __restrict__ seed_in, const GridParams* __restrict__ seed_lattice) {
  const uint32_t i_raw = blockIdx.x * blockDim.x + threadIdx.x;
  const bool LANE_VALID = i_raw < n_q;
  const uint32_t i = min(i_raw, n_q - 1u);
  const float4 q = qsorted[i];
  const f3 p = mk3(q.x, q.y, q.z);
  Best<MODE> best;
  if (mesh.n_nodes) {
    const float scale = fmaxf(mesh_scale(mesh), fmaxf(fabsf(p.x), fmaxf(fabsf(p.y), fabsf(p.z))));
    const float slack = 4.0e-6f * scale + (MODE == MODE_NORMAL_FOLD ? 2.5e-6f : 0.0f);
    uint32_t slot = 0;
    if (seed_in != nullptr) slot = min(seed_in[query_lattice_cell(*seed_lattice, p.x, p.y, p.z)], mesh.n_tris - 1);
    eval_triangle<MODE>(best, p, mesh.tris[slot]);
    greedy_leaf<MODE>(mesh, p, best);
    uint32_t st_nodes = 0, st_exact = 0;
    __shared__ LaneShare lane_share[4];
    lane_tree_walk<MODE>(mesh, p, slack, best, LANE_VALID, st_nodes, st_exact, lane_share[threadIdx.x >> 6]);
    if (mesh.stats != nullptr && LANE_VALID) {
      atomicAdd(&mesh.stats[0], (unsigned long long)st_nodes);
      atomicAdd(&mesh.stats[2], (unsigned long long)st_exact);
      atomicAdd(&mesh.stats[3], 1ull);
      atomicMax(&mesh.stats[72], (unsigned long long)st_nodes);
      atomicMax(&mesh.stats[73], (unsigned long long)st_exact);
    }
  }
  bool negate = false;
  if (MODE == MODE_UNSIGNED && SIGN == SIGN_RAYS3) {
    const uint32_t cx = stab_count_lane<0>(mesh, p), cy = stab_count_lane<1>(mesh, p);
    uint32_t cz = cx;
    if (((cx ^ cy) & 1u) != 0u) cz = stab_count_lane<2>(mesh, p);
    negate = ((cx & 1u) + (cy & 1u) + (cz & 1u)) > 1u;
  }
  if (!LANE_VALID) return;
  if (MODE == MODE_NORMAL_FOLD && best.nan) atomicOr(err, ERRF_NAN);
  out[perm[i]] = finish<MODE>(best, negate);
}


struct PacketArgs {
  DeviceMesh mesh{};
  GridParams g{};
  const float4* qsorted = nullptr;
  const uint32_t *perm = nullptr, *plane = nullptr;
  uint32_t n_q = 0, n_packets = 0;
  float* out = nullptr;
  int* err = nullptr;
  const uint32_t* seed_in = nullptr;
  uint32_t seed_shift = 0, seed_ny = 0, seed_nz = 0;
  const GridParams* seed_lattice = nullptr;
  CutList cut = {nullptr, 0, 0, 0, 0, nullptr};
  PeerOut peers{};
  SplitCtl split{};
};
template <bool GRID, int MODE, int SIGN>
void launch_packet(hipStream_t st, const PacketArgs& a, int defer) {
  const uint32_t per = 8u << XCD_RUN_LOG;
  const uint32_t grid_blocks = ((a.n_packets + per - 1) / per) * per;
  const auto launch = [&](auto stats, auto split, auto form) {
    hipLaunchKernelGGL((k_packet<GRID, MODE, SIGN, decltype(stats)::value, decltype(split)::value, decltype(form)::value>), dim3(grid_blocks), dim3(64), 0, st,
                       a.mesh, a.g, a.qsorted, a.perm, a.n_q, a.plane, a.out, a.err, a.n_packets, a.seed_in, a.seed_shift, a.seed_ny, a.seed_nz, a.seed_lattice,
                       a.cut, a.peers, a.split);
  };
  constexpr std::true_type yes{};
  constexpr std::false_type no{};
  constexpr std::integral_constant<int, 0> f0{};
  constexpr std::integral_constant<int, 1> f1{};
  constexpr std::integral_constant<int, 2> f2{};
  constexpr std::integral_constant<int, 3> f3{};
#ifdef M2S_STATS_BUILD
  if (a.mesh.stats != nullptr) return launch(yes, no, f0);
#endif
  if constexpr (GRID && MODE != MODE_NEAREST_NORMAL)
    if (a.split.cnt != nullptr) return defer == 3 ? launch(no, yes, f3) : launch(no, yes, f1);
  if constexpr (GRID)
    if (defer == 2) return launch(no, no, f2);
  return defer == 3 ? launch(no, no, f3) : defer ? launch(no, no, f1) : launch(no, no, f0);
}
template <int MODE, int SIGN>
void launch_split_rounds(hipStream_t st, const DeviceMesh& mesh, const GridParams& g, const uint32_t* plane, float* out, int* err,
                         const SplitCtl& split, const CutList& cut, const PeerOut& peers) {
  constexpr unsigned waves = 16384;
  const bool trace = tuning().split_report >= 2;
  if (trace) { const hipError_t e = hipStreamSynchronize(st); fprintf(stderr, "[m2s split] packet launch: %s\n", hipGetErrorString(e)); }
  for (uint32_t r = 1; r <= split.rounds; ++r) {
    hipLaunchKernelGGL((k_split_round<MODE>), dim3(waves), dim3(64), 0, st, mesh, g, split, cut, r, r == split.rounds, err);
    if (trace) { const hipError_t e = hipStreamSynchronize(st); fprintf(stderr, "[m2s split] round %u: %s\n", r, hipGetErrorString(e)); }
  }
  hipLaunchKernelGGL((k_split_finish<MODE, SIGN>), dim3(2048), dim3(256), 0, st, g, plane, out, split, peers);
  if (trace) { const hipError_t e = hipStreamSynchronize(st); fprintf(stderr, "[m2s split] finish: %s\n", hipGetErrorString(e)); }
}

uint32_t host_brick_count(const GridParams& g) { return brick_counts(g).padded; }

}

constexpr uint32_t SPLIT_MAX_PACKETS = 1u << 19, SPLIT_ITEMS_PER_SLOT = 8;
static uint32_t split_cap_slots(size_t packets) { return (uint32_t)std::min<size_t>(std::max<size_t>(packets, 64), SPLIT_MAX_PACKETS); }
static uint32_t split_patience_q8(uint32_t packets, const Tuning& tn) {
  const double rounds_before = std::max(1.0, (double)packets / 8192.0 - 1.0);
  return (uint32_t)std::min(65535.0 * 256.0, 256.0 * tn.split_patience / rounds_before);
}

GridWalkChoice choose_grid_walk(const GridParams& g, size_t n_tris, size_t n_nodes, uint32_t leaf_max, bool counting, int algorithm, const Tuning& tn) {
  GridWalkChoice ch;
  if (slab_is_empty(g)) return ch;
  const BrickCounts bc = brick_counts(g);
  const uint32_t packets = bc.padded;
  const bool interleaved = g.chunk_log < 31u;
  if ((n_nodes == 0 && n_tris != 0 && algorithm == 0) || grid_is_tiny(g, n_tris, algorithm, true, tn)) {
    ch.path = GridWalkChoice::ALL_PAIRS_SPLIT;
    return ch;
  }
  const bool brute = algorithm == 1;
  ch.seeds = grid_walk_wants_seeds(g, n_tris, algorithm);
  const int lane_env = tn.lane_walk;
  const double real_bricks = (double)bc.real, grid_bricks = (double)bc.grid;
  const bool split_possible = !brute && n_nodes != 0 && tn.split != 0 && !counting && packets <= SPLIT_MAX_PACKETS;
  const bool split_auto = split_possible && tn.split < 0 && real_bricks >= 10240.0 && n_tris >= 300000u && (double)n_tris >= 5.0 * grid_bricks;
  const double lane_ratio = split_auto ? tn.lane_ratio_split : tn.lane_ratio;
  const bool lane_walk = !brute && n_tris && (lane_env >= 0 ? lane_env == 1 : (leaf_max <= 2u && (double)n_tris > lane_ratio * real_bricks));
  const uint32_t cut_min_packets = tn.cut_min_packets;
  if (!brute && !lane_walk && ch.seeds && packets >= cut_min_packets) {
    const int cc = tn.cut_coarse;
    const size_t waves = cut_blocks(g, 2);
    const bool blocks_ok = !interleaved || g.chunk_log >= g.bl[0] + 2u;
    const bool two_level = blocks_ok && (cc > 0 || (cc < 0 && waves >= tn.cut_coarse_min_waves));
    ch.cut_levels = two_level ? 2 : 1;
  }
  const int gk = tn.group;
  const bool can = !brute && !lane_walk && ch.cut_levels == 0 && n_nodes != 0 && !counting && tn.split <= 0 && !split_auto && tn.defer < 0 && !interleaved;
  const bool want = gk > 0 || (gk < 0 && (double)n_tris >= tn.group_min_ratio * real_bricks);
  if (can && want) {
    uint32_t w = 1;
    while (w < GROUP_MAX_WAVES && (double)(2u * w) * real_bricks <= (double)tn.group_target_waves) w *= 2;
    if (gk > 0 && w < 2u) w = GROUP_MAX_WAVES;
    if (w >= 2u) ch.group_waves = w;
  }
  ch.split = !lane_walk && split_possible && ch.group_waves == 0 && (tn.split > 0 || split_auto);
  ch.split_forced = ch.split && tn.split == 2;
  ch.defer = tn.defer == 0 ? 0 : tn.defer > 0 ? tn.defer : ((double)n_tris < 0.02 * grid_bricks ? 2 : (double)n_tris < 0.045 * grid_bricks ? 1 : 3);
  ch.path = lane_walk ? GridWalkChoice::LANE : ch.group_waves ? GridWalkChoice::GROUP : brute ? GridWalkChoice::ALL_PAIRS : GridWalkChoice::PACKET;
  return ch;
}
GridWalkChoice choose_grid_walk_for_sizing(const GridParams& g, size_t n_tris) { return choose_grid_walk(g, n_tris, 1, ~0u, false, 0, tuning()); }

static size_t split_workspace_bytes(const GridParams& g, size_t n_tris, size_t packets) {
  if (!choose_grid_walk_for_sizing(g, n_tris).split) return 0;
  const size_t cap = split_cap_slots(packets);
  const size_t items = std::max<size_t>(cap, std::min<size_t>(cap * SPLIT_ITEMS_PER_SLOT, 1u << 20));
  const size_t rounds = std::min(tuning().split_rounds, SPLIT_MAX_ROUNDS);
  return 256 + SPLIT_CNT_WORDS * 4 + cap * 4 + 256 + cap * 128 * 4 + 256 + rounds * items * 16 + 256;
}
size_t grid_distance_workspace_bytes(const GridParams& g, size_t n_tris) {
  const BrickCounts bc = brick_counts(g);
  const size_t bricks = (size_t)bc.padded;
  if ((double)(g.xe - g.xb) * g.n[1] * g.n[2] <= 4194304.0)
    return bricks * 44 + bricks + 16384 + cut_blocks(g, 0) * CUT_WORDS * 4 + cut_blocks(g, 2) * CUTC_S * CUTC_WORDS * 4 + 512 + TOP_SUBTREES * 8 + 256 + bricks * 64 * 8 + 4096 + split_workspace_bytes(g, n_tris, bricks);
  const size_t trail_counters = (size_t)bc.nb[0] * (bc.nb[1] + 1) * 4;
  return bricks * 44 + bricks + 16384 + cut_blocks(g, 0) * CUT_WORDS * 4 + cut_blocks(g, 2) * CUTC_S * CUTC_WORDS * 4 + 512 + TOP_SUBTREES * 8 + 256 + trail_counters + 1024 + split_workspace_bytes(g, n_tris, bricks);
}

uint32_t host_packet_bricks(const GridParams& g) { return slab_is_empty(g) ? 0u : host_brick_count(g); }
bool grid_walk_wants_seeds(const GridParams& g, size_t n_tris, int algorithm) { return algorithm != 1 && n_tris && host_packet_bricks(g) >= 8; }

int prepare_grid_walk(Arena& ws, hipStream_t st, const DeviceMesh& mesh, const GridParams& g, int algorithm, bool pipelined,
                      GridWalkPlan* plan, const SeedLattice* raw_seeds) {
  *plan = GridWalkPlan{};
  const Tuning& tn = tuning();
  const GridWalkChoice ch = choose_grid_walk(g, mesh.n_tris, mesh.n_nodes, mesh.leaf_max, mesh.stats != nullptr, algorithm, tn);
  plan->choice = ch;
  if (ch.path == GridWalkChoice::NOTHING) return 0;
  const BrickCounts bc = brick_counts(g);
  const uint32_t packets = bc.padded;
  if (ch.path == GridWalkChoice::ALL_PAIRS_SPLIT) {
    plan->brute_acc = ws.take<uint32_t>((size_t)packets * 64 * 2);
    if (!plan->brute_acc) { set_error("internal: brute-force workspace too small"); return M2S_ERR_HIP_INTERNAL; }
    return 0;
  }
  if (ch.seeds) {
    SeedLattice lat;
    if (raw_seeds && raw_seeds->ids) {
      lat = *raw_seeds;
      launch_seed_remap(st, lat.ids, lat.points, mesh.slot_of, mesh.n_tris);
    } else {
      const int rc = launch_grid_seeds(ws, st, mesh.cen, mesh.n_tris, g, &lat);
      if (rc) return rc;
    }
    plan->seeds = lat.ids; plan->seed_shift = lat.shift; plan->seed_ny = lat.ny; plan->seed_nz = lat.nz;
  }
  if (ch.cut_levels) {
    uint32_t* lists = ws.take<uint32_t>((size_t)bc.real * CUT_WORDS);
    if (!lists) { set_error("internal: cut-list workspace too small"); return M2S_ERR_HIP_INTERNAL; }
    uint32_t* coarse = nullptr;
    if (ch.cut_levels == 2) {
      coarse = ws.take<uint32_t>(cut_blocks(g, 2) * CUTC_S * CUTC_WORDS);
      if (!coarse) { set_error("internal: cut-list workspace too small"); return M2S_ERR_HIP_INTERNAL; }
    }
    launch_grid_cut(st, mesh, g, plan->seeds, plan->seed_shift, plan->seed_ny, plan->seed_nz, lists, coarse);
    plan->cut_lists = lists; plan->cut_log = 0; plan->cut_ny = bc.nb[1]; plan->cut_nz = bc.nb[2];
  }
  if (ch.path == GridWalkChoice::GROUP) {
    uint2* top = ws.take<uint2>(TOP_SUBTREES);
    if (!top) { set_error("internal: workspace too small"); return M2S_ERR_HIP_INTERNAL; }
    hipLaunchKernelGGL(k_tree_top, dim3(1), dim3(TOP_SUBTREES), 0, st, mesh, top);
    plan->group_top = top;
  }
  if (ch.split) {
    SplitCtl sc;
    sc.cap_slots = split_cap_slots(packets);
    sc.cap_items = std::max(sc.cap_slots, std::min(sc.cap_slots * SPLIT_ITEMS_PER_SLOT, 1u << 20));
    sc.rounds = std::min(tn.split_rounds, SPLIT_MAX_ROUNDS);
    sc.emit_min = std::max(2u, tn.split_min_records) * (uint32_t)sizeof(NodeExt);
    sc.emit_max = std::max(std::max(2u, tn.split_min_records), tn.split_max_records) * (uint32_t)sizeof(NodeExt);
    sc.grace = tn.split_budget ? tn.split_budget : 128u;
    sc.idle_below = ch.split_forced ? 1u : 0u;
    sc.patience_q8 = split_patience_q8(packets, tn);
    sc.cnt = ws.take<uint32_t>(SPLIT_CNT_WORDS);
    sc.slot_packet = ws.take<uint32_t>(sc.cap_slots);
    sc.acc = ws.take<uint32_t>((size_t)sc.cap_slots * 128);
    sc.items = ws.take<uint4>((size_t)sc.rounds * sc.cap_items);
    if (!sc.cnt || !sc.slot_packet || !sc.acc || !sc.items) { set_error("internal: split-walk workspace too small"); return M2S_ERR_HIP_INTERNAL; }
    plan->split = sc;
  }
  return 0;
}

int launch_grid_walk(hipStream_t st, const DeviceMesh& mesh, const GridParams& g, int mode, const uint32_t* d_inside_plane,
                     const GridWalkPlan& plan, uint32_t bx_off, float* d_out, int* d_err, const PeerOut* peers) {
  const GridWalkChoice& ch = plan.choice;
  if (slab_is_empty(g) || ch.path == GridWalkChoice::NOTHING) return 0;
  PeerOut pz{};
  if (peers) pz = *peers;
  const BrickCounts bc = brick_counts(g);
  const uint32_t packets = bc.padded, real = (uint32_t)bc.real;
  const uint32_t* plane = mode == MODE_UNSIGNED ? d_inside_plane : nullptr;
  const CutList cut = {plan.cut_lists, plan.cut_log, plan.cut_ny, plan.cut_nz, bx_off, nullptr};
  if (ch.path == GridWalkChoice::ALL_PAIRS_SPLIT) {
    M2S_HIP_CHECK(hipMemsetD32Async((hipDeviceptr_t)plan.brute_acc, 0x7f800000, (size_t)packets * 64 * 2, st));
    return launch_grid_brute_split(st, mesh, g, mode, plane, plan.brute_acc, real, d_out, d_err, pz);
  }
  if (ch.path == GridWalkChoice::ALL_PAIRS) return launch_grid_brute(st, mesh, g, mode, plane, d_out, d_err, packets, pz);
  const bool split = ch.path == GridWalkChoice::PACKET && ch.split && (mode != MODE_NORMAL_FOLD || tuning().split > 0);
  PacketArgs a;
  a.mesh = mesh; a.g = g; a.plane = plane; a.out = d_out; a.err = d_err; a.n_packets = packets;
  a.seed_in = plan.seeds; a.seed_shift = plan.seed_shift; a.seed_ny = plan.seed_ny; a.seed_nz = plan.seed_nz; a.cut = cut; a.peers = pz;
  if (split) {
    a.split = plan.split;
    if (!ch.split_forced) a.split.patience_q8 = split_patience_q8(packets, tuning());
    hipLaunchKernelGGL(k_split_init, dim3(1), dim3(64), 0, st, a.split.cnt, ch.split_forced ? 1u : 0u);
  }
  for_grid_form(mode, plane != nullptr, [&](auto form) {
    constexpr int MODE = decltype(form)::MODE, SIGN = decltype(form)::SIGN;
    switch (ch.path) {
      case GridWalkChoice::NOTHING: case GridWalkChoice::ALL_PAIRS_SPLIT: case GridWalkChoice::ALL_PAIRS: break;
      case GridWalkChoice::LANE:
        hipLaunchKernelGGL((k_lane<MODE, SIGN>), dim3((packets + 3) / 4), dim3(256), 0, st, mesh, g, plane, d_out, d_err, packets, a.seed_in, a.seed_shift, a.seed_ny, a.seed_nz, bx_off, pz);
        break;
      case GridWalkChoice::GROUP: {
        const uint32_t per = 8u << XCD_RUN_LOG, grid_blocks = ((packets + per - 1) / per) * per;
        const size_t lds = ((size_t)ch.group_waves * 256u + DeferLayout<MODE>::SLOT_WORDS) * 4u;
        hipLaunchKernelGGL((k_packet_group<MODE, SIGN>), dim3(grid_blocks), dim3(64 * ch.group_waves), lds, st, mesh, g, plane, d_out, d_err, packets,
                           a.seed_in, a.seed_shift, a.seed_ny, a.seed_nz, bx_off, plan.group_top, pz);
        break;
      }
      case GridWalkChoice::PACKET:
        launch_packet<true, MODE, SIGN>(st, a, ch.defer);
        if (split) launch_split_rounds<MODE, SIGN>(st, mesh, g, plane, d_out, d_err, a.split, cut, pz);
        break;
    }
  });
  M2S_HIP_CHECK(hipGetLastError());
  if (split && tuning().split_report) {
    const SplitCtl& sc = a.split;
    uint32_t h[SPLIT_CNT_WORDS];
    M2S_HIP_CHECK(hipStreamSynchronize(st));
    M2S_HIP_CHECK(hipMemcpy(h, sc.cnt, sizeof(h), hipMemcpyDeviceToHost));
    fprintf(stderr, "[m2s split] %u packets: %u suspended (room for %u); items per round:", packets, h[0], sc.cap_slots);
    for (uint32_t r = 1; r <= sc.rounds; ++r) fprintf(stderr, " %u", h[1 + r]);
    fprintf(stderr, " (room for %u each, reserved in blocks of 64); first look after %u units, patience %.2f of the time to the flag, subtrees of %u .. %u records; XCD 0: handed out in %.1f us\n",
            sc.cap_items, sc.grace, sc.patience_q8 / 256.0, sc.emit_min / (uint32_t)sizeof(NodeExt), sc.emit_max / (uint32_t)sizeof(NodeExt),
            h[16] ? ((h[16] & ~1u) - h[24]) * 0.01 : 0.0);
  }
  return 0;
}

int launch_grid_distance(Arena& ws, hipStream_t st, const DeviceMesh& mesh, const GridParams& g, int mode,
                         const uint32_t* d_inside_plane, int algorithm, float* d_out, int* d_err,
                         hipEvent_t ev_before_final, hipEvent_t wait_before_final, bool pipelined,
                         const SeedLattice* raw_seeds, hipEvent_t wait_raw_seeds, const PeerOut* peers) {
  GridWalkPlan plan;
  if (raw_seeds && wait_raw_seeds) M2S_HIP_CHECK(hipStreamWaitEvent(st, wait_raw_seeds, 0));
  int rc = prepare_grid_walk(ws, st, mesh, g, algorithm, pipelined, &plan, raw_seeds);
  if (rc) return rc;
  if (wait_before_final) M2S_HIP_CHECK(hipStreamWaitEvent(st, wait_before_final, 0));
  if (ev_before_final) M2S_HIP_CHECK(hipEventRecord(ev_before_final, st));
  return launch_grid_walk(st, mesh, g, mode, d_inside_plane, plan, 0, d_out, d_err, peers);
}

bool query_walk_is_lane(size_t n_q, size_t n_tris, int sign_src) {
  const int lane_env = tuning().lane_walk;
  return n_tris && sign_src != SIGN_XRAY_ALL && (lane_env >= 0 ? lane_env == 1 : (double)n_q < tuning().query_lane_coeff * (double)n_tris);
}
uint32_t query_leaf_max(size_t n_q, size_t n_tris, int sign_src) {
  const Tuning& tn = tuning();
  if (tn.leaf_max != 0) return tn.leaf_max;
  if (n_tris == 0 || query_walk_is_lane(n_q, n_tris, sign_src)) return 2u;
  const double per_tri = (double)n_q / (double)n_tris;
  return per_tri < 50.0 ? 8u : per_tri < 500.0 ? 4u : 2u;
}

uint32_t grid_leaf_max(const GridParams& g, size_t n_tris) {
  const Tuning& tn = tuning();
  if (tn.leaf_max != 0) return tn.leaf_max;
  const double per_brick = (double)n_tris / std::max(1.0, (double)brick_counts(g).grid);
  return per_brick >= 40.0 ? 16u : per_brick >= 3.0 ? 8u : per_brick >= 0.6 ? 4u : 2u;
}

int launch_query_walk(Arena& ws, hipStream_t st, const DeviceMesh& mesh, const float* d_queries, const QueryPlan& plan,
                      int mode, int sign_src, int algorithm, float* d_out, int* d_err, const QuerySeeds* pre) {
  const size_t n_q = plan.n_q;
  if (n_q == 0) return 0;
  GridParams g{};
  const uint32_t nq = (uint32_t)n_q;
  if (algorithm == 1) return launch_query_brute(st, mesh, d_queries, nq, mode, sign_src, d_out, d_err);
  const uint32_t launched = plan.launched;
  const uint32_t* seeds = nullptr;
  const GridParams* d_lat = nullptr;
  if (plan.seeds && mesh.n_tris) {
    QuerySeeds own;
    if (pre == nullptr || pre->ids == nullptr) {
      const int rc = launch_query_seeds(ws, st, mesh.cen, mesh.n_tris, plan, false, &own);
      if (rc) return rc;
      pre = &own;
    } else if (pre->raw) {
      launch_seed_remap(st, pre->ids, (size_t)QL * QL * QL, mesh.slot_of, mesh.n_tris);
    }
    seeds = pre->ids;
    d_lat = plan.lat;
  }
  CutList cut = {nullptr, 0, 0, 0, 0, nullptr};
  if (plan.centres != nullptr && seeds != nullptr) {
    uint32_t* lists = ws.take<uint32_t>((size_t)launched * CUT_WORDS);
    if (!lists) { set_error("internal: query workspace too small"); return M2S_ERR_HIP_INTERNAL; }
    launch_query_cut(st, mesh, seeds, launched, lists, plan.centres, plan.table, d_lat);
    cut = {lists, 0, 0, 0, 0, plan.centres};
  }
  PacketArgs a;
  a.mesh = mesh; a.g = g; a.qsorted = plan.sorted; a.perm = plan.perm; a.n_q = nq; a.plane = plan.table; a.out = d_out; a.err = d_err; a.n_packets = launched;
  a.seed_in = seeds; a.seed_lattice = d_lat; a.cut = cut;
  const int defer = tuning().defer == 0 ? 0 : tuning().defer == 1 ? 1 : 3;
  for_query_form(mode, sign_src, [&](auto form) {
    constexpr int MODE = decltype(form)::MODE, SIGN = decltype(form)::SIGN;
    if (plan.lane_walk) hipLaunchKernelGGL((k_lane_q<MODE, SIGN>), dim3((nq + 255u) / 256u), dim3(256), 0, st, mesh, a.qsorted, a.perm, nq, d_out, d_err, seeds, d_lat);
    else launch_packet<false, MODE, SIGN>(st, a, defer);
  });
  M2S_HIP_CHECK(hipGetLastError());
  return 0;
}

int launch_query_distance(Arena& ws, hipStream_t st, const DeviceMesh& mesh, const float* d_queries, size_t n_q,
                          int mode, int sign_src, int algorithm, float* d_out, int* d_err) {
  if (query_is_tiny(n_q, mesh.n_tris, algorithm, sign_src) && mesh.stats == nullptr)
    return launch_query_brute_split(ws, st, mesh, d_queries, n_q, mode, sign_src, d_out, d_err);
  QueryPlan plan;
  const int rc = prepare_query_walk(ws, st, d_queries, n_q, mesh.n_tris, sign_src, algorithm, &plan, nullptr);
  if (rc) return rc;
  return launch_query_walk(ws, st, mesh, d_queries, plan, mode, sign_src, algorithm, d_out, d_err, nullptr);
}

__global__ void k_warm_distance() {}
void warm_distance(hipStream_t st) {
  hipLaunchKernelGGL(k_warm_distance, dim3(1), dim3(64), 0, st);
  const void* fns[] = {
      (const void*)k_packet<true, MODE_UNSIGNED, SIGN_GRID_PLANE, false, false, 3>,
      (const void*)k_packet<true, MODE_UNSIGNED, SIGN_GRID_PLANE, false, false, 2>,
      (const void*)k_packet<true, MODE_NORMAL_FOLD, SIGN_NONE, false, false, 3>,
      (const void*)k_packet<true, MODE_NORMAL_FOLD, SIGN_NONE, false, false, 2>,
      (const void*)k_packet<false, MODE_UNSIGNED, SIGN_RAYS3, false, false, 3>,
      (const void*)k_packet<false, MODE_NEAREST_NORMAL, SIGN_NONE, false, false, 3>,
      (const void*)k_split_init,
      (const void*)k_split_round<MODE_UNSIGNED>,
      (const void*)k_split_round<MODE_NORMAL_FOLD>,
      (const void*)k_split_finish<MODE_UNSIGNED, SIGN_GRID_PLANE>,
      (const void*)k_split_finish<MODE_NORMAL_FOLD, SIGN_NONE>,
      (const void*)k_lane<MODE_UNSIGNED, SIGN_GRID_PLANE>,
      (const void*)k_lane_q<MODE_UNSIGNED, SIGN_RAYS3>};
  hipFuncAttributes attr;
  for (const void* f : fns) (void)hipFuncGetAttributes(&attr, f);
  (void)hipGetLastError();
}

}
```

### mesh_to_sdf_amd/csrc/walk.hip.h

```cpp
#pragma once
#include "common.h"
#include "geo.hip.h"

namespace m2s {

namespace {

constexpr float F32_MAX_C = 3.402823466e+38f;

template <class T>
__device__ __forceinline__ T record_at_bytes(const void* base, uint32_t byte_offset) {
  static_assert(sizeof(T) % 16 == 0 && alignof(T) >= 16, "records are whole 16-byte words");
  typedef uint32_t u32x4 __attribute__((ext_vector_type(4)));
  typedef uint32_t u32x8 __attribute__((ext_vector_type(8), aligned(16)));
  typedef uint32_t u32x16 __attribute__((ext_vector_type(16), aligned(16)));
  typedef const __attribute__((address_space(4))) char* const_bytes;
  const const_bytes q = (const_bytes)(uintptr_t)base + byte_offset;
  constexpr unsigned N16 = sizeof(T) / 64, R16 = sizeof(T) % 64, N8 = R16 / 32, N4 = (R16 % 32) / 16;
  union { T rec; unsigned char raw[sizeof(T)]; } u;
#pragma unroll
  for (unsigned k = 0; k < N16; ++k) { const u32x16 v = *(const __attribute__((address_space(4))) u32x16*)(q + 64 * k); __builtin_memcpy(u.raw + 64 * k, &v, 64); }
#pragma unroll
  for (unsigned k = 0; k < N8; ++k) { const u32x8 v = *(const __attribute__((address_space(4))) u32x8*)(q + 64 * N16 + 32 * k); __builtin_memcpy(u.raw + 64 * N16 + 32 * k, &v, 32); }
#pragma unroll
  for (unsigned k = 0; k < N4; ++k) { const u32x4 v = *(const __attribute__((address_space(4))) u32x4*)(q + 64 * N16 + 32 * N8 + 16 * k); __builtin_memcpy(u.raw + 64 * N16 + 32 * N8 + 16 * k, &v, 16); }
  return u.rec;
}
template <class T>
__device__ __forceinline__ T record_at(const T* base, uint32_t index) {
  return record_at_bytes<T>(base, index * (uint32_t)sizeof(T));
}

template <class T>
__device__ __forceinline__ T record_at_vec(const T* base, uint32_t uniform_index) {
  uint32_t vi;
  asm("v_mov_b32_e32 %0, %1" : "=v"(vi) : "s"(uniform_index));
  return *reinterpret_cast<const T*>(reinterpret_cast<const char*>(base) + (size_t)vi * sizeof(T));
}

struct GridBrick {
  uint32_t x, y, z;
  uint32_t bx, by, bz;
  bool in_range;
  bool brick_in_grid;
};

__host__ __device__ __forceinline__ uint32_t bricks_along(uint32_t cells, uint32_t log2_extent) {
  return (cells + (1u << log2_extent) - 1u) >> log2_extent;
}
__host__ __device__ __forceinline__ uint32_t super_brick_xlog(uint32_t nbx, uint32_t xl_cap = 0) {
  for (uint32_t xl = xl_cap ? xl_cap - 1u : 3u; xl > 0; --xl) {
    const uint32_t padded = ((nbx + (1u << xl) - 1u) >> xl) << xl;
    if ((padded - nbx) * 8u <= nbx) return xl;
  }
  return 0;
}
__device__ __forceinline__ uint32_t div_magic(uint32_t n, uint32_t d, uint32_t magic) {
  return magic ? __umulhi(n, magic) : n / d;
}
__device__ __forceinline__ void brick_coords(const GridParams& g, uint32_t brick, uint32_t* bx, uint32_t* by, uint32_t* bz) {
  const uint32_t nby = bricks_along(g.n[1], g.bl[1]), nbz = bricks_along(g.n[2], g.bl[2]);
  const uint32_t sy = (nby + 7) >> 3, sz = (nbz + 7) >> 3;
  const uint32_t xl = super_brick_xlog(bricks_along(g.xe - g.xb, g.bl[0]), g.xl_cap);
  const uint32_t sb = brick >> (6 + xl), in = brick & ((64u << xl) - 1u);
  const uint32_t t = div_magic(sb, sz, g.sz_magic), sbz = sb - t * sz;
  const uint32_t sbx = div_magic(t, sy, g.sy_magic), sby = t - sbx * sy;
  *bx = (sbx << xl) + (in >> 6);
  *by = sby * 8 + ((in >> 3) & 7u);
  *bz = sbz * 8 + (in & 7u);
}
__device__ __forceinline__ GridBrick grid_lane_voxel(const GridParams& g, uint32_t brick, int lane) {
  uint32_t bx, by, bz;
  brick_coords(g, brick, &bx, &by, &bz);
  GridBrick v;
  const uint32_t lx = g.bl[0], ly = g.bl[1], lz = g.bl[2], l = (uint32_t)lane;
  const uint32_t layers = g.xe - g.xb, xv = (bx << lx) + (l >> (ly + lz));
  v.y = (by << ly) + ((l >> lz) & ((1u << ly) - 1u));
  v.z = (bz << lz) + (l & ((1u << lz) - 1u));
  v.in_range = xv < layers && v.y < g.n[1] && v.z < g.n[2];
  v.brick_in_grid = ((bx << lx) < layers) && ((by << ly) < g.n[1]) && ((bz << lz) < g.n[2]);
  v.bx = bx; v.by = by; v.bz = bz;
  v.x = slab_x(g, min(xv, layers - 1u));
  v.y = min(v.y, g.n[1] - 1);
  v.z = min(v.z, g.n[2] - 1);
  return v;
}
__device__ __forceinline__ f3 grid_point(const GridParams& g, const GridBrick& v) {
  return {cell_center(g.first[0], g.size[0], v.x), cell_center(g.first[1], g.size[1], v.y),
          cell_center(g.first[2], g.size[2], v.z)};
}
__device__ __forceinline__ uint32_t grid_brick_count(const GridParams& g) {
  return bricks_along(g.xe - g.xb, g.bl[0]) * bricks_along(g.n[1], g.bl[1]) * bricks_along(g.n[2], g.bl[2]);
}

__device__ __forceinline__ GridBrick grid_lane_voxel_plain(const GridParams& g, uint32_t brick, int lane) {
  const uint32_t nby = bricks_along(g.n[1], g.bl[1]), nbz = bricks_along(g.n[2], g.bl[2]);
  const uint32_t bz = brick % nbz, t = brick / nbz, by = t % nby, bx = t / nby;
  GridBrick v;
  const uint32_t lx = g.bl[0], ly = g.bl[1], lz = g.bl[2], l = (uint32_t)lane;
  const uint32_t layers = g.xe - g.xb, xv = (bx << lx) + (l >> (ly + lz));
  v.y = (by << ly) + ((l >> lz) & ((1u << ly) - 1u));
  v.z = (bz << lz) + (l & ((1u << lz) - 1u));
  v.in_range = xv < layers && v.y < g.n[1] && v.z < g.n[2];
  v.brick_in_grid = true;
  v.bx = bx; v.by = by; v.bz = bz;
  v.x = slab_x(g, min(xv, layers - 1u));
  v.y = min(v.y, g.n[1] - 1);
  v.z = min(v.z, g.n[2] - 1);
  return v;
}

#ifndef M2S_XCD_RUN_LOG
#define M2S_XCD_RUN_LOG 8
#endif
constexpr uint32_t XCD_RUN_LOG = M2S_XCD_RUN_LOG;
__device__ __forceinline__ uint32_t xcd_remap(uint32_t b) {
  const uint32_t i = b >> 3, x = b & 7u;
  return ((((i >> XCD_RUN_LOG) << 3) + x) << XCD_RUN_LOG) | (i & ((1u << XCD_RUN_LOG) - 1u));
}

template <int MODE>
struct Best {
  float d2 = __builtin_inff();
  float d2pos = __builtin_inff();
  uint32_t idx = 0xffffffffu;
  bool pos = false;
  bool nan = false;
};

template <int MODE>
__device__ __forceinline__ void eval_triangle(Best<MODE>& best, f3 p, const TriRec& tr) {
  const f3 a = mk3(tr.ax, tr.ay, tr.az), b = mk3(tr.bx, tr.by, tr.bz), c = mk3(tr.cx, tr.cy, tr.cz);
  const TriEdges e = {mk3(tr.abx, tr.aby, tr.abz), mk3(tr.acx, tr.acy, tr.acz), mk3(tr.bcx, tr.bcy, tr.bcz)};
  const uint32_t cls = tr.cls, index = tr.index;
  if (MODE == MODE_UNSIGNED) {
    const float d2 = point_triangle_dist2(p, a, b, c, e, cls);
    best.d2 = fminf(best.d2, d2);
  } else {
    bool positive;
    const float d2 = point_triangle_dist2_signed_n(p, a, b, c, e, cls, mk3(tr.nrx, tr.nry, tr.nrz), &positive);
    if (MODE == MODE_NORMAL_FOLD) {
      best.nan |= !(d2 == d2);
      best.d2 = fminf(best.d2, d2);
      if (positive) best.d2pos = fminf(best.d2pos, d2);
    } else {
      if (d2 < best.d2 || (d2 == best.d2 && index < best.idx)) { best.d2 = d2; best.idx = index; best.pos = positive; }
    }
  }
}

template <int MODE>
__device__ __forceinline__ void eval_triangle_leaf(Best<MODE>& best, f3 p, const TriRec& tr, bool reach) {
  if (MODE == MODE_NEAREST_NORMAL || tr.cls != TRI_REGULAR) { eval_triangle<MODE>(best, p, tr); return; }
  const f3 a = mk3(tr.ax, tr.ay, tr.az), b = mk3(tr.bx, tr.by, tr.bz), c = mk3(tr.cx, tr.cy, tr.cz);
  const f3 ab = mk3(tr.abx, tr.aby, tr.abz), ac = mk3(tr.acx, tr.acy, tr.acz);
  const RegularHead h = closest_point_regular_head(p, a, b, c, ab, ac);
  const bool vertex = h.rA | h.rB | h.rC;
  f3 q;
  bool valid = true;
  if (__ballot(reach & !vertex) == 0ull) {
    q = closest_point_regular_vertex(h, a, b, c);
    valid = vertex;
  } else {
    q = closest_point_regular_tail(h, a, b, c, ab, ac, mk3(tr.bcx, tr.bcy, tr.bcz));
  }
  const f3 d = sub3(p, q);
  float d2 = dot3(d, d);
  if (MODE == MODE_UNSIGNED) {
    d2 = valid ? d2 : __builtin_inff();
    best.d2 = fminf(best.d2, d2);
  } else {
    const bool positive = dot3(d, mk3(tr.nrx, tr.nry, tr.nrz)) > 0.0f;
    best.nan |= valid & !(d2 == d2);
    d2 = valid ? d2 : __builtin_inff();
    best.d2 = fminf(best.d2, d2);
    if (positive) best.d2pos = fminf(best.d2pos, d2);
  }
}

template <int MODE>
__device__ __forceinline__ float finish(const Best<MODE>& best, bool negate_unsigned) {
  if (MODE == MODE_UNSIGNED) {
    const float d = fminf(F32_MAX_C, sqrtf(best.d2));
    return negate_unsigned ? -d : d;
  }
  if (MODE == MODE_NORMAL_FOLD) return normal_fold_result(best.d2, best.d2pos);
  const float d = sqrtf(best.d2);
  return best.pos ? d : -d;
}

constexpr float PRUNE_REL = 4.0e-6f;
__device__ __forceinline__ float prune_bound(float best_d2, float slack) {
  const float d = __builtin_amdgcn_sqrtf(best_d2);
  const float r = __builtin_fmaf(d, 1.0f + PRUNE_REL, slack);
  return r * r;
}

__device__ __forceinline__ float box_dist2(f3 p, float mnx, float mny, float mnz, float mxx, float mxy, float mxz) {
  const float dx = fmaxf(fmaxf(mnx - p.x, p.x - mxx), 0.0f);
  const float dy = fmaxf(fmaxf(mny - p.y, p.y - mxy), 0.0f);
  const float dz = fmaxf(fmaxf(mnz - p.z, p.z - mxz), 0.0f);
  return __builtin_fmaf(dx, dx, __builtin_fmaf(dy, dy, dz * dz));
}

__device__ __forceinline__ float ext_dist2(f3 p, const NodeExt& e) {
  const float vx = p.x - e.cx, vy = p.y - e.cy, vz = p.z - e.cz;
  const float t = __builtin_fmaf(e.nz, vz, __builtin_fmaf(e.ny, vy, e.nx * vx));
  const float v2 = __builtin_fmaf(vz, vz, __builtin_fmaf(vy, vy, vx * vx));
  const float l2 = __builtin_fmaf(-1.0e-6f, v2, __builtin_fmaf(-t, t, v2));
  const float lat = fmaxf(__builtin_amdgcn_sqrtf(l2) - e.R, 0.0f);
  const float s = fmaxf(fabsf(t - e.mid) - e.half, 0.0f);
  return __builtin_fmaf(s, s, lat * lat);
}

__device__ __forceinline__ float planes_dist2(f3 p, const TriPlanes& t) {
  const float h = __builtin_fmaf(t.nz, p.z, __builtin_fmaf(t.ny, p.y, t.nx * p.x)) - t.dn;
  const float e0 = __builtin_fmaf(t.m0z, p.z, __builtin_fmaf(t.m0y, p.y, t.m0x * p.x)) - t.o0;
  const float e1 = __builtin_fmaf(t.m1z, p.z, __builtin_fmaf(t.m1y, p.y, t.m1x * p.x)) - t.o1;
  const float e2 = __builtin_fmaf(t.m2z, p.z, __builtin_fmaf(t.m2y, p.y, t.m2x * p.x)) - t.o2;
  const float e = fmaxf(fmaxf(e0, e1), fmaxf(e2, 0.0f));
  return __builtin_fmaf(h, h, e * e);
}

}

}
```

Baseline: 17720 Mvoxels/s.

## Precompute packet kernel constants on host and hoist cut/seed/sign loads early

Adds a host-computed PacketConsts block holding brick-decode, cut-list decode and delivery constants, passed to the packet kernels so they no longer re-derive super-brick counts and cut bit masks per wave. In k_packet the cut-list word, seed word and sign-plane word are loaded at kernel entry, behind a scheduling barrier, so their latency overlaps the seed-triangle evaluation instead of stalling later. Plain-delivery stores also skip the peer-store path. This costs more kernel arguments and keeps a few extra registers live across the seed evaluation, which may affect occupancy. It also adds debug hooks for the packet constants and brick decode.

```diff
diff --git a/mesh_to_sdf_amd/csrc/capi.hip b/mesh_to_sdf_amd/csrc/capi.hip
--- a/mesh_to_sdf_amd/csrc/capi.hip
+++ b/mesh_to_sdf_amd/csrc/capi.hip
@@ -2553,4 +2553,32 @@
   return m2s_debug_grid_walk_choice_slab(grid, nullptr, n_tris, n_nodes, leaf_max, algorithm, out);
 }
 
-}
+
+int m2s_debug_packet_consts(const uint32_t n[3], uint32_t xb, uint32_t xe, const uint32_t bl[3], uint32_t xl_cap, uint32_t n_nodes, const uint32_t shape[7],
+                            uint32_t out[28]) {
+  g_err[0] = 0;
+  if (!n || !bl || !out) return fail(M2S_ERR_BAD_ARG, "NULL argument");
+  if (xb > xe || xe > n[0] || bl[0] + bl[1] + bl[2] != 6u || n_nodes > (1u << 27) + 64u) return fail(M2S_ERR_BAD_ARG, "bad slab, brick or tree");
+  GridParams g{};
+  for (int a = 0; a < 3; ++a) { g.n[a] = n[a]; g.bl[a] = bl[a]; g.size[a] = 1.0f; }
+  g.xb = xb; g.xe = xe; g.nzw = (n[2] + 31u) / 32u; g.xl_cap = xl_cap; g.chunk_log = 31; g.period = 0;
+  g.out_off = (uint64_t)xb * n[1] * n[2];
+  set_super_brick_magic(g);
+  const uint32_t zero[7] = {0, 0, 0, 0, 0, 0, 0};
+  const uint32_t* s = shape ? shape : zero;
+  const PacketConsts k = packet_consts(g, n_nodes, s[0], s[1], s[2], s[3], s[4], s[5], s[6], nullptr);
+  static_assert(sizeof(k) == 28 * sizeof(uint32_t), "the hook's word count");
+  memcpy(out, &k, sizeof(k));
+  return M2S_OK;
+}
+int m2s_debug_packet_bricks(const uint32_t consts[28], uint32_t first, uint32_t count, uint32_t* out) {
+  g_err[0] = 0;
+  if (!consts || (!out && count)) return fail(M2S_ERR_BAD_ARG, "NULL argument");
+  PacketConsts k;
+  memcpy(&k, consts, sizeof(k));
+  if (k.sy == 0u || k.sz == 0u || k.xl > 3u) return fail(M2S_ERR_BAD_ARG, "not a block of m2s_debug_packet_consts");
+  for (uint32_t i = 0; i < count; ++i) packet_brick(k, first + i, out + 3 * (size_t)i);
+  return M2S_OK;
+}
+
+}
diff --git a/mesh_to_sdf_amd/csrc/common.h b/mesh_to_sdf_amd/csrc/common.h
--- a/mesh_to_sdf_amd/csrc/common.h
+++ b/mesh_to_sdf_amd/csrc/common.h
@@ -81,10 +81,12 @@
   return g.xb + (v >> g.chunk_log) * g.period + (v & ((1u << g.chunk_log) - 1u));
 }
 
+__host__ __device__ __forceinline__ uint32_t super_bricks_along(uint32_t bricks) { return (bricks + 7) >> 3; }
+
 inline void set_super_brick_magic(GridParams& g) {
   const uint64_t nbx = (g.n[0] + (1u << g.bl[0]) - 1u) >> g.bl[0], nby = (g.n[1] + (1u << g.bl[1]) - 1u) >> g.bl[1],
                  nbz = (g.n[2] + (1u << g.bl[2]) - 1u) >> g.bl[2];
-  const uint64_t sy = (nby + 7) >> 3, sz = (nbz + 7) >> 3, n_max = (nbx + 1) * sy * sz;
+  const uint64_t sy = super_bricks_along((uint32_t)nby), sz = super_bricks_along((uint32_t)nbz), n_max = (nbx + 1) * sy * sz;
   const uint64_t d_max = sy > sz ? sy : sz;
   const bool safe = n_max * d_max < (1ull << 32);
   g.sz_magic = (safe && sz > 1) ? (uint32_t)(((1ull << 32) + sz - 1) / sz) : 0u;
@@ -120,6 +122,20 @@
   uint32_t units;
   uint32_t* progress;
 };
+
+struct PacketConsts {
+  uint32_t cut_S, cut_mask, cut_len_bits, cut_len_mask;
+  uint32_t n_nodes, tree_end_bytes;
+  uint32_t xl, sy, sz, sy_magic, sz_magic;
+  uint32_t nbx, nby, nbz, layers;
+  uint32_t seed_shift, seed_ny, seed_nz;
+  uint32_t cut_log, cut_ny, cut_nz, bx_off;
+  uint32_t nzw, n1, n2;
+  uint32_t delivery;
+  uint64_t out_off;
+};
+enum : uint32_t { DELIVER_PLAIN = 0, DELIVER_PEER_STORE = 1, DELIVER_TRAIL = 2 };
+static_assert(sizeof(PacketConsts) == 28 * 4 && sizeof(PacketConsts) % 8 == 0, "PacketConsts: 26 words and one 64-bit offset");
 
 enum : int { ERRF_INDEX_OOB = 1, ERRF_NAN = 2, ERRF_TRAIL_TIMEOUT = 4, ERRF_BUILD_TIMEOUT = 8, ERRF_SPLIT_OVERFLOW = 16 };
 
@@ -257,6 +273,9 @@
                       GridWalkPlan* plan, const SeedLattice* raw_seeds = nullptr);
 int launch_grid_walk(hipStream_t st, const DeviceMesh& mesh, const GridParams& g, int mode, const uint32_t* d_inside_plane,
                      const GridWalkPlan& plan, uint32_t bx_off, float* d_out, int* d_err, const PeerOut* peers = nullptr);
+PacketConsts packet_consts(const GridParams& g, uint32_t n_nodes, uint32_t seed_shift, uint32_t seed_ny, uint32_t seed_nz, uint32_t cut_log,
+                           uint32_t cut_ny, uint32_t cut_nz, uint32_t bx_off, const PeerOut* peers);
+void packet_brick(const PacketConsts& k, uint32_t packet, uint32_t brick[3]);
 int launch_push_cells(hipStream_t st, const float* src, const PeerOut& peers, uint64_t first, uint64_t count);
 uint32_t trail_unit_log(const GridParams& g);
 uint32_t trail_units(const GridParams& g);
diff --git a/mesh_to_sdf_amd/csrc/dist.hip.h b/mesh_to_sdf_amd/csrc/dist.hip.h
--- a/mesh_to_sdf_amd/csrc/dist.hip.h
+++ b/mesh_to_sdf_amd/csrc/dist.hip.h
@@ -26,10 +26,23 @@
 static_assert(M2S_CUT_MAX <= 15, "the range count has four bits");
 struct CutList {
   const uint32_t* lists;
-  uint32_t log, ny, nz;
-  uint32_t bx_off;
   const float4* centres;
 };
+__device__ __forceinline__ uint32_t cut_block_of(const PacketConsts& k, const GridBrick& vox) {
+  return (((vox.bx + k.bx_off) >> k.cut_log) * k.cut_ny + (vox.by >> k.cut_log)) * k.cut_nz + (vox.bz >> k.cut_log);
+}
+__device__ __forceinline__ uint32_t seed_point_of(const PacketConsts& k, const GridBrick& vox) {
+  return (((vox.bx + k.bx_off) >> k.seed_shift) * k.seed_ny + (vox.by >> k.seed_shift)) * k.seed_nz + (vox.bz >> k.seed_shift);
+}
+__device__ __forceinline__ size_t sign_word_index(const PacketConsts& k, const GridBrick& vox) {
+  return ((size_t)vox.x * k.n1 + vox.y) * k.nzw + (vox.z >> 5);
+}
+__device__ __forceinline__ void cut_decode_ranges(const PacketConsts& k, uint32_t cw, uint32_t* off_v, uint32_t* end_v) {
+  const uint32_t cfirst = cw & k.cut_mask;
+  const uint32_t clen = ((cw >> k.cut_S) & k.cut_len_mask) << (cw >> 27);
+  *off_v = cfirst * (uint32_t)sizeof(NodeExt);
+  *end_v = min(cfirst + clen, k.n_nodes) * (uint32_t)sizeof(NodeExt);
+}
 constexpr uint32_t CUTC_S_LOG = 3, CUTC_S = 1u << CUTC_S_LOG, CUTC_WORDS = 8, CUTC_MAX = CUTC_WORDS - 1;
 static_assert(CUTC_S * CUTC_WORDS == 64, "a fine wave fetches its block's coarse record with one load, lane = word");
 
@@ -85,7 +98,7 @@
   c.real = (uint64_t)c.nb[0] * c.nb[1] * c.nb[2];
   c.grid = (uint64_t)bricks_along(g.n[0], g.bl[0]) * c.nb[1] * c.nb[2];
   const uint32_t xl = super_brick_xlog(c.nb[0], g.xl_cap);
-  c.padded = ((c.nb[0] + (1u << xl) - 1u) >> xl) * ((c.nb[1] + 7) >> 3) * ((c.nb[2] + 7) >> 3) * (64u << xl);
+  c.padded = ((c.nb[0] + (1u << xl) - 1u) >> xl) * super_bricks_along(c.nb[1]) * super_bricks_along(c.nb[2]) * (64u << xl);
   return c;
 }
 static size_t cut_blocks(const GridParams& g, uint32_t log) {
diff --git a/mesh_to_sdf_amd/csrc/distance.hip b/mesh_to_sdf_amd/csrc/distance.hip
--- a/mesh_to_sdf_amd/csrc/distance.hip
+++ b/mesh_to_sdf_amd/csrc/distance.hip
@@ -417,12 +417,11 @@
 }
 
 template <bool GRID, int MODE, int SIGN, bool STATS, bool SPLIT, int DEFER = 0>
-__global__ __launch_bounds__(64) __attribute__((amdgpu_waves_per_eu(8, 8))) void k_packet(DeviceMesh mesh, GridParams g, const float4* __restrict__ qsorted,
+__global__ __launch_bounds__(64) __attribute__((amdgpu_waves_per_eu(8, 8))) void k_packet(PacketConsts k, DeviceMesh mesh, GridParams g, const float4* __restrict__ qsorted,
                                                const uint32_t* __restrict__ perm, uint32_t n_q,
                                                const uint32_t* __restrict__ plane, float* __restrict__ out,
                                                int* __restrict__ err, uint32_t n_packets,
-                                               const uint32_t* __restrict__ seed_in, uint32_t seed_shift,
-                                               uint32_t seed_ny, uint32_t seed_nz,
+                                               const uint32_t* __restrict__ seed_in,
                                                const GridParams* __restrict__ seed_lattice, CutList cut, PeerOut peers, SplitCtl split) {
   const int lane = threadIdx.x & 63;
   if (SPLIT && (blockIdx.x < 8u || blockIdx.x + 8u >= gridDim.x) && lane == 0) {
@@ -438,64 +437,59 @@
   size_t out_index;
   bool store;
   GridBrick vox{};
+  uint32_t cw = 0, seed_word = 0, sign_word = 0;
+  const bool walks = k.n_nodes != 0u, listed = walks && cut.lists != nullptr, seeded = walks && seed_in != nullptr;
+  float tree_scale = 0.0f;
   if (GRID) {
-    vox = grid_lane_voxel(g, packet, lane);
+    vox = grid_lane_voxel(g, k, packet, lane);
     if (!vox.brick_in_grid) return;
+    if (!walks && MODE == MODE_UNSIGNED && SIGN == SIGN_GRID_PLANE) sign_word = plane[sign_word_index(k, vox)];
+    if (listed) cw = cut.lists[(size_t)__builtin_amdgcn_readfirstlane(cut_block_of(k, vox)) * CUT_WORDS + ((uint32_t)lane & 15u)];
+    if (seeded) seed_word = seed_in[seed_point_of(k, vox)];
+    __builtin_amdgcn_sched_barrier(0);
     p = grid_point(g, vox);
-    out_index = ((size_t)vox.x * g.n[1] + vox.y) * g.n[2] + vox.z - (size_t)g.out_off;
+    out_index = ((size_t)vox.x * k.n1 + vox.y) * k.n2 + vox.z - (size_t)k.out_off;
     store = vox.in_range;
   } else {
     uint32_t first, cnt;
     if (!query_packet_range(plane, packet, n_q, &first, &cnt)) return;
+    if (listed) {
+      cw = cut.lists[(size_t)packet * CUT_WORDS + ((uint32_t)lane & 15u)];
+    }
+    if (walks) tree_scale = mesh_scale(mesh);
     const uint32_t i = first + min((uint32_t)lane, cnt - 1u);
     const float4 q = qsorted[i];
     p = mk3(q.x, q.y, q.z);
     out_index = perm[i];
     store = (uint32_t)lane < cnt;
+    if (seeded) {
+      const GridParams L = *seed_lattice;
+      float q0[3] = {__shfl(p.x, 0), __shfl(p.y, 0), __shfl(p.z, 0)};
+      if (cut.centres != nullptr) {
+        const float4 c = cut.centres[packet];
+        q0[0] = c.x; q0[1] = c.y; q0[2] = c.z;
+      }
+      seed_word = seed_in[__builtin_amdgcn_readfirstlane(query_lattice_cell(L, q0[0], q0[1], q0[2]))];
+    }
   }
 
   Best<MODE> best;
   WalkStats st;
   uint32_t st_ranges = 0, st_band = 0, st_rbytes = 0;
-  if (mesh.n_nodes) {
-    const float scale = fmaxf(mesh_scale(mesh), fmaxf(fabsf(p.x), fmaxf(fabsf(p.y), fabsf(p.z))));
-    const float slack = 4.0e-6f * scale + (MODE == MODE_NORMAL_FOLD ? 2.5e-6f : 0.0f);
+  if (walks) {
     SplitState sp;
     if (SPLIT) split_arm(sp, split, 0u, true);
     __shared__ unsigned long long defer_lds[DEFER ? DeferLayout<MODE>::DWORDS : 1];
     DeferQueue dq = {nullptr, nullptr, 0u, 0u};
     if (DEFER) dq = defer_begin<MODE>(defer_lds);
 
-    constexpr uint32_t NB = (uint32_t)sizeof(NodeExt);
-    const uint32_t* cl = nullptr;
-    uint32_t n_ranges = 1, cut_off_v = 0, cut_end_v = (lane == 1) ? mesh.n_nodes * NB : 0u;
-    if (SPLIT) sp.n_ranges = &n_ranges;
-    if (cut.lists != nullptr) {
-      const uint32_t cb = GRID ? __builtin_amdgcn_readfirstlane((((vox.bx + cut.bx_off) >> cut.log) * cut.ny + (vox.by >> cut.log)) * cut.nz + (vox.bz >> cut.log))
-                               : packet;
-      cl = cut.lists + (size_t)cb * CUT_WORDS;
-      const uint32_t cw = cl[(uint32_t)lane & 15u];
-      const uint32_t cS = cut_start_bits(mesh.n_nodes), cfirst = cw & ((1u << cS) - 1u);
-      const uint32_t clen = ((cw >> cS) & ((1u << (27u - cS)) - 1u)) << (cw >> 27);
-      cut_off_v = cfirst * NB;
-      cut_end_v = min(cfirst + clen, mesh.n_nodes) * NB;
-      n_ranges = __builtin_amdgcn_readfirstlane(cw);
-    }
-    if (seed_in != nullptr) {
-      uint32_t sidx = packet;
+    if (seeded) {
+      const uint32_t slot = __builtin_amdgcn_readfirstlane(min(seed_word, mesh.n_tris - 1));
+      const TriRec tr = record_at(mesh.tris, slot);
       if (GRID) {
-        sidx = (((vox.bx + cut.bx_off) >> seed_shift) * seed_ny + (vox.by >> seed_shift)) * seed_nz + (vox.bz >> seed_shift);
-      } else {
-        const GridParams L = *seed_lattice;
-        float q0[3] = {__shfl(p.x, 0), __shfl(p.y, 0), __shfl(p.z, 0)};
-        if (cut.centres != nullptr) {
-          const float4 c = cut.centres[packet];
-          q0[0] = c.x; q0[1] = c.y; q0[2] = c.z;
-        }
-        sidx = __builtin_amdgcn_readfirstlane(query_lattice_cell(L, q0[0], q0[1], q0[2]));
-      }
-      const uint32_t slot = __builtin_amdgcn_readfirstlane(min(seed_in[sidx], mesh.n_tris - 1));
-      const TriRec tr = record_at(mesh.tris, slot);
+        tree_scale = mesh_scale(mesh);
+        if (MODE == MODE_UNSIGNED && SIGN == SIGN_GRID_PLANE) sign_word = plane[sign_word_index(k, vox)];
+      }
       eval_triangle<MODE>(best, p, tr);
     } else {
       const f3 c = {__shfl(p.x, 0), __shfl(p.y, 0), __shfl(p.z, 0)};
@@ -513,7 +507,21 @@
         nr = go_left ? nl : nrr;
       }
       const TriRec tr = mesh.tris[nr.tri];
+      if (GRID) {
+        tree_scale = mesh_scale(mesh);
+        if (MODE == MODE_UNSIGNED && SIGN == SIGN_GRID_PLANE) sign_word = plane[sign_word_index(k, vox)];
+      }
       eval_triangle<MODE>(best, p, tr);
+    }
+    const float scale = fmaxf(tree_scale, fmaxf(fabsf(p.x), fmaxf(fabsf(p.y), fabsf(p.z))));
+    const float slack = 4.0e-6f * scale + (MODE == MODE_NORMAL_FOLD ? 2.5e-6f : 0.0f);
+    __builtin_amdgcn_sched_barrier(0);
+
+    uint32_t n_ranges = 1, cut_off_v = 0, cut_end_v = (lane == 1) ? k.tree_end_bytes : 0u;
+    if (SPLIT) sp.n_ranges = &n_ranges;
+    if (listed) {
+      cut_decode_ranges(k, cw, &cut_off_v, &cut_end_v);
+      n_ranges = __builtin_amdgcn_readfirstlane(cw);
     }
 
     float thr = prune_bound(best.d2, slack);
@@ -571,8 +579,7 @@
   bool negate = false;
   if (MODE == MODE_UNSIGNED) {
     if (SIGN == SIGN_GRID_PLANE) {
-      const size_t w = ((size_t)vox.x * g.n[1] + vox.y) * g.nzw + (vox.z >> 5);
-      negate = (plane[w] >> (vox.z & 31u)) & 1u;
+      negate = (sign_word >> (vox.z & 31u)) & 1u;
     } else if (SIGN == SIGN_RAYS3) {
       __shared__ uint32_t ray_lds[DEFER != 0 ? 192 : 1];
       const uint32_t cx = DEFER != 0 ? stab_count_dense<0>(mesh, p, ray_lds) : stab_count<0>(mesh, p);
@@ -584,7 +591,7 @@
   }
   if (MODE == MODE_NORMAL_FOLD && best.nan) atomicOr(err, ERRF_NAN);
   const float result = finish<MODE>(best, negate);
-  if (GRID) store_grid_result(out, out_index, result, store, g, vox, peers, lane);
+  if (GRID && k.delivery != DELIVER_PLAIN) store_grid_result(out, out_index, result, store, g, vox, peers, lane);
   else if (store) out[out_index] = result;
 }
 
@@ -606,13 +613,13 @@
 template <int MODE, int SIGN>
 __global__ __launch_bounds__(64 * GROUP_MAX_WAVES) __attribute__((amdgpu_waves_per_eu(8, 8))) void k_packet_group(
     DeviceMesh mesh, GridParams g, const uint32_t* __restrict__ plane, float* __restrict__ out, int* __restrict__ err, uint32_t n_packets,
-    const uint32_t* __restrict__ seed_in, uint32_t seed_shift, uint32_t seed_ny, uint32_t seed_nz, uint32_t bx_off, const uint2* __restrict__ top, PeerOut peers) {
+    const uint32_t* __restrict__ seed_in, PacketConsts k, const uint2* __restrict__ top, PeerOut peers) {
   static_assert(MODE == MODE_UNSIGNED || MODE == MODE_NORMAL_FOLD, "grid modes");
   const int lane = threadIdx.x & 63;
   const uint32_t wave = (uint32_t)__builtin_amdgcn_readfirstlane((int)(threadIdx.x >> 6));
   const uint32_t packet = (uint32_t)__builtin_amdgcn_readfirstlane((int)xcd_remap(blockIdx.x));
   if (packet >= n_packets) return;
-  const GridBrick vox = grid_lane_voxel(g, packet, lane);
+  const GridBrick vox = grid_lane_voxel(g, k, packet, lane);
   if (!vox.brick_in_grid) return;
   const f3 p = grid_point(g, vox);
   const size_t out_index = ((size_t)vox.x * g.n[1] + vox.y) * g.n[2] + vox.z - (size_t)g.out_off;
@@ -631,8 +638,7 @@
     const float slack = 4.0e-6f * scale + (MODE == MODE_NORMAL_FOLD ? 2.5e-6f : 0.0f);
     uint32_t slot = 0;
     if (seed_in != nullptr) {
-      const uint32_t sidx = (((vox.bx + bx_off) >> seed_shift) * seed_ny + (vox.by >> seed_shift)) * seed_nz + (vox.bz >> seed_shift);
-      slot = __builtin_amdgcn_readfirstlane(min(seed_in[sidx], mesh.n_tris - 1));
+      slot = __builtin_amdgcn_readfirstlane(min(seed_in[seed_point_of(k, vox)], mesh.n_tris - 1));
     }
     eval_triangle<MODE>(best, p, record_at(mesh.tris, slot));
     float thr = prune_bound(best.d2, slack);
@@ -668,9 +674,8 @@
 }
 
 template <int MODE>
-__global__ __launch_bounds__(64) __attribute__((amdgpu_waves_per_eu(8, 8))) void k_split_round(DeviceMesh mesh, GridParams g, SplitCtl split, CutList cut, uint32_t round, bool final, int* __restrict__ err) {
+__global__ __launch_bounds__(64) __attribute__((amdgpu_waves_per_eu(8, 8))) void k_split_round(PacketConsts k, DeviceMesh mesh, GridParams g, SplitCtl split, CutList cut, uint32_t round, bool final, int* __restrict__ err) {
   constexpr uint32_t AW = MODE == MODE_NORMAL_FOLD ? 128u : 64u;
-  constexpr uint32_t NB = (uint32_t)sizeof(NodeExt);
   const int lane = threadIdx.x & 63;
   const uint32_t n_items = min(split.cnt[1u + round], split.cap_items);
   const uint4* list = split.items + (size_t)(round - 1u) * split.cap_items;
@@ -681,7 +686,7 @@
     const bool continuation = (tag & SPLIT_CONTINUATION) != 0u;
     uint32_t off = __builtin_amdgcn_readfirstlane(it.y);
     if (!continuation && off >= third) continue;
-    const GridBrick vox = grid_lane_voxel(g, packet, lane);
+    const GridBrick vox = grid_lane_voxel(g, k, packet, lane);
     const f3 p = grid_point(g, vox);
     const float scale = fmaxf(mesh_scale(mesh), fmaxf(fabsf(p.x), fmaxf(fabsf(p.y), fabsf(p.z))));
     const float slack = 4.0e-6f * scale + (MODE == MODE_NORMAL_FOLD ? 2.5e-6f : 0.0f);
@@ -699,14 +704,10 @@
     wave_lds_sync();
     DeferQueue dq = defer_begin<MODE>(defer_lds);
     if (continuation) {
-      uint32_t n_ranges = 1, cut_off_v = 0, cut_end_v = (lane == 1) ? mesh.n_nodes * NB : 0u;
+      uint32_t n_ranges = 1, cut_off_v = 0, cut_end_v = (lane == 1) ? k.tree_end_bytes : 0u;
       if (cut.lists != nullptr) {
-        const uint32_t cb = __builtin_amdgcn_readfirstlane((((vox.bx + cut.bx_off) >> cut.log) * cut.ny + (vox.by >> cut.log)) * cut.nz + (vox.bz >> cut.log));
-        const uint32_t cw = cut.lists[(size_t)cb * CUT_WORDS + ((uint32_t)lane & 15u)];
-        const uint32_t cS = cut_start_bits(mesh.n_nodes), cfirst = cw & ((1u << cS) - 1u);
-        const uint32_t clen = ((cw >> cS) & ((1u << (27u - cS)) - 1u)) << (cw >> 27);
-        cut_off_v = cfirst * NB;
-        cut_end_v = min(cfirst + clen, mesh.n_nodes) * NB;
+        const uint32_t cw = cut.lists[(size_t)__builtin_amdgcn_readfirstlane(cut_block_of(k, vox)) * CUT_WORDS + ((uint32_t)lane & 15u)];
+        cut_decode_ranges(k, cw, &cut_off_v, &cut_end_v);
         n_ranges = __builtin_amdgcn_readfirstlane(cw);
       }
       if (!final) emit_begin(em, split, round + 1u, packet, slot);
@@ -1003,6 +1004,7 @@
 
 
 struct PacketArgs {
+  PacketConsts k{};
   DeviceMesh mesh{};
   GridParams g{};
   const float4* qsorted = nullptr;
@@ -1011,9 +1013,8 @@
   float* out = nullptr;
   int* err = nullptr;
   const uint32_t* seed_in = nullptr;
-  uint32_t seed_shift = 0, seed_ny = 0, seed_nz = 0;
   const GridParams* seed_lattice = nullptr;
-  CutList cut = {nullptr, 0, 0, 0, 0, nullptr};
+  CutList cut = {nullptr, nullptr};
   PeerOut peers{};
   SplitCtl split{};
 };
@@ -1023,8 +1024,7 @@
   const uint32_t grid_blocks = ((a.n_packets + per - 1) / per) * per;
   const auto launch = [&](auto stats, auto split, auto form) {
     hipLaunchKernelGGL((k_packet<GRID, MODE, SIGN, decltype(stats)::value, decltype(split)::value, decltype(form)::value>), dim3(grid_blocks), dim3(64), 0, st,
-                       a.mesh, a.g, a.qsorted, a.perm, a.n_q, a.plane, a.out, a.err, a.n_packets, a.seed_in, a.seed_shift, a.seed_ny, a.seed_nz, a.seed_lattice,
-                       a.cut, a.peers, a.split);
+                       a.k, a.mesh, a.g, a.qsorted, a.perm, a.n_q, a.plane, a.out, a.err, a.n_packets, a.seed_in, a.seed_lattice, a.cut, a.peers, a.split);
   };
   constexpr std::true_type yes{};
   constexpr std::false_type no{};
@@ -1042,13 +1042,13 @@
   return defer == 3 ? launch(no, no, f3) : defer ? launch(no, no, f1) : launch(no, no, f0);
 }
 template <int MODE, int SIGN>
-void launch_split_rounds(hipStream_t st, const DeviceMesh& mesh, const GridParams& g, const uint32_t* plane, float* out, int* err,
+void launch_split_rounds(hipStream_t st, const DeviceMesh& mesh, const GridParams& g, const PacketConsts& k, const uint32_t* plane, float* out, int* err,
                          const SplitCtl& split, const CutList& cut, const PeerOut& peers) {
   constexpr unsigned waves = 16384;
   const bool trace = tuning().split_report >= 2;
   if (trace) { const hipError_t e = hipStreamSynchronize(st); fprintf(stderr, "[m2s split] packet launch: %s\n", hipGetErrorString(e)); }
   for (uint32_t r = 1; r <= split.rounds; ++r) {
-    hipLaunchKernelGGL((k_split_round<MODE>), dim3(waves), dim3(64), 0, st, mesh, g, split, cut, r, r == split.rounds, err);
+    hipLaunchKernelGGL((k_split_round<MODE>), dim3(waves), dim3(64), 0, st, k, mesh, g, split, cut, r, r == split.rounds, err);
     if (trace) { const hipError_t e = hipStreamSynchronize(st); fprintf(stderr, "[m2s split] round %u: %s\n", r, hipGetErrorString(e)); }
   }
   hipLaunchKernelGGL((k_split_finish<MODE, SIGN>), dim3(2048), dim3(256), 0, st, g, plane, out, split, peers);
@@ -1057,6 +1057,31 @@
 
 uint32_t host_brick_count(const GridParams& g) { return brick_counts(g).padded; }
 
+}
+
+PacketConsts packet_consts(const GridParams& g, uint32_t n_nodes, uint32_t seed_shift, uint32_t seed_ny, uint32_t seed_nz, uint32_t cut_log,
+                           uint32_t cut_ny, uint32_t cut_nz, uint32_t bx_off, const PeerOut* peers) {
+  PacketConsts k{};
+  k.cut_S = cut_start_bits(n_nodes);
+  k.cut_mask = (1u << k.cut_S) - 1u;
+  k.cut_len_bits = 27u - k.cut_S;
+  k.cut_len_mask = (1u << k.cut_len_bits) - 1u;
+  k.n_nodes = n_nodes;
+  k.tree_end_bytes = n_nodes * (uint32_t)sizeof(NodeExt);
+  k.layers = g.xe - g.xb;
+  k.nbx = bricks_along(k.layers, g.bl[0]), k.nby = bricks_along(g.n[1], g.bl[1]), k.nbz = bricks_along(g.n[2], g.bl[2]);
+  k.xl = super_brick_xlog(k.nbx, g.xl_cap);
+  k.sy = super_bricks_along(k.nby), k.sz = super_bricks_along(k.nbz);
+  k.sy_magic = g.sy_magic, k.sz_magic = g.sz_magic;
+  k.seed_shift = seed_shift, k.seed_ny = seed_ny, k.seed_nz = seed_nz;
+  k.cut_log = cut_log, k.cut_ny = cut_ny, k.cut_nz = cut_nz, k.bx_off = bx_off;
+  k.nzw = g.nzw, k.n1 = g.n[1], k.n2 = g.n[2];
+  k.delivery = peers == nullptr ? DELIVER_PLAIN : peers->progress != nullptr ? DELIVER_TRAIL : peers->n != 0u ? DELIVER_PEER_STORE : DELIVER_PLAIN;
+  k.out_off = g.out_off;
+  return k;
+}
+void packet_brick(const PacketConsts& k, uint32_t packet, uint32_t brick[3]) {
+  brick_coords_in(k.xl, k.sy, k.sz, k.sy_magic, k.sz_magic, packet, &brick[0], &brick[1], &brick[2]);
 }
 
 constexpr uint32_t SPLIT_MAX_PACKETS = 1u << 19, SPLIT_ITEMS_PER_SLOT = 8;
@@ -1199,7 +1224,7 @@
   const BrickCounts bc = brick_counts(g);
   const uint32_t packets = bc.padded, real = (uint32_t)bc.real;
   const uint32_t* plane = mode == MODE_UNSIGNED ? d_inside_plane : nullptr;
-  const CutList cut = {plan.cut_lists, plan.cut_log, plan.cut_ny, plan.cut_nz, bx_off, nullptr};
+  const CutList cut = {plan.cut_lists, nullptr};
   if (ch.path == GridWalkChoice::ALL_PAIRS_SPLIT) {
     M2S_HIP_CHECK(hipMemsetD32Async((hipDeviceptr_t)plan.brute_acc, 0x7f800000, (size_t)packets * 64 * 2, st));
     return launch_grid_brute_split(st, mesh, g, mode, plane, plan.brute_acc, real, d_out, d_err, pz);
@@ -1208,7 +1233,8 @@
   const bool split = ch.path == GridWalkChoice::PACKET && ch.split && (mode != MODE_NORMAL_FOLD || tuning().split > 0);
   PacketArgs a;
   a.mesh = mesh; a.g = g; a.plane = plane; a.out = d_out; a.err = d_err; a.n_packets = packets;
-  a.seed_in = plan.seeds; a.seed_shift = plan.seed_shift; a.seed_ny = plan.seed_ny; a.seed_nz = plan.seed_nz; a.cut = cut; a.peers = pz;
+  a.seed_in = plan.seeds; a.cut = cut; a.peers = pz;
+  a.k = packet_consts(g, mesh.n_nodes, plan.seed_shift, plan.seed_ny, plan.seed_nz, plan.cut_log, plan.cut_ny, plan.cut_nz, bx_off, &pz);
   if (split) {
     a.split = plan.split;
     if (!ch.split_forced) a.split.patience_q8 = split_patience_q8(packets, tuning());
@@ -1219,18 +1245,18 @@
     switch (ch.path) {
       case GridWalkChoice::NOTHING: case GridWalkChoice::ALL_PAIRS_SPLIT: case GridWalkChoice::ALL_PAIRS: break;
       case GridWalkChoice::LANE:
-        hipLaunchKernelGGL((k_lane<MODE, SIGN>), dim3((packets + 3) / 4), dim3(256), 0, st, mesh, g, plane, d_out, d_err, packets, a.seed_in, a.seed_shift, a.seed_ny, a.seed_nz, bx_off, pz);
+        hipLaunchKernelGGL((k_lane<MODE, SIGN>), dim3((packets + 3) / 4), dim3(256), 0, st, mesh, g, plane, d_out, d_err, packets, a.seed_in, plan.seed_shift, plan.seed_ny, plan.seed_nz, bx_off, pz);
         break;
       case GridWalkChoice::GROUP: {
         const uint32_t per = 8u << XCD_RUN_LOG, grid_blocks = ((packets + per - 1) / per) * per;
         const size_t lds = ((size_t)ch.group_waves * 256u + DeferLayout<MODE>::SLOT_WORDS) * 4u;
         hipLaunchKernelGGL((k_packet_group<MODE, SIGN>), dim3(grid_blocks), dim3(64 * ch.group_waves), lds, st, mesh, g, plane, d_out, d_err, packets,
-                           a.seed_in, a.seed_shift, a.seed_ny, a.seed_nz, bx_off, plan.group_top, pz);
+                           a.seed_in, a.k, plan.group_top, pz);
         break;
       }
       case GridWalkChoice::PACKET:
         launch_packet<true, MODE, SIGN>(st, a, ch.defer);
-        if (split) launch_split_rounds<MODE, SIGN>(st, mesh, g, plane, d_out, d_err, a.split, cut, pz);
+        if (split) launch_split_rounds<MODE, SIGN>(st, mesh, g, a.k, plane, d_out, d_err, a.split, cut, pz);
         break;
     }
   });
@@ -1303,16 +1329,17 @@
     seeds = pre->ids;
     d_lat = plan.lat;
   }
-  CutList cut = {nullptr, 0, 0, 0, 0, nullptr};
+  CutList cut = {nullptr, nullptr};
   if (plan.centres != nullptr && seeds != nullptr) {
     uint32_t* lists = ws.take<uint32_t>((size_t)launched * CUT_WORDS);
     if (!lists) { set_error("internal: query workspace too small"); return M2S_ERR_HIP_INTERNAL; }
     launch_query_cut(st, mesh, seeds, launched, lists, plan.centres, plan.table, d_lat);
-    cut = {lists, 0, 0, 0, 0, plan.centres};
+    cut = {lists, plan.centres};
   }
   PacketArgs a;
   a.mesh = mesh; a.g = g; a.qsorted = plan.sorted; a.perm = plan.perm; a.n_q = nq; a.plane = plan.table; a.out = d_out; a.err = d_err; a.n_packets = launched;
   a.seed_in = seeds; a.seed_lattice = d_lat; a.cut = cut;
+  a.k = packet_consts(g, mesh.n_nodes, 0, 0, 0, 0, 0, 0, 0, nullptr);
   const int defer = tuning().defer == 0 ? 0 : tuning().defer == 1 ? 1 : 3;
   for_query_form(mode, sign_src, [&](auto form) {
     constexpr int MODE = decltype(form)::MODE, SIGN = decltype(form)::SIGN;
diff --git a/mesh_to_sdf_amd/csrc/walk.hip.h b/mesh_to_sdf_amd/csrc/walk.hip.h
--- a/mesh_to_sdf_amd/csrc/walk.hip.h
+++ b/mesh_to_sdf_amd/csrc/walk.hip.h
@@ -55,26 +55,42 @@
   }
   return 0;
 }
-__device__ __forceinline__ uint32_t div_magic(uint32_t n, uint32_t d, uint32_t magic) {
+__host__ __device__ __forceinline__ uint32_t div_magic(uint32_t n, uint32_t d, uint32_t magic) {
+#if defined(__HIP_DEVICE_COMPILE__)
   return magic ? __umulhi(n, magic) : n / d;
-}
-__device__ __forceinline__ void brick_coords(const GridParams& g, uint32_t brick, uint32_t* bx, uint32_t* by, uint32_t* bz) {
-  const uint32_t nby = bricks_along(g.n[1], g.bl[1]), nbz = bricks_along(g.n[2], g.bl[2]);
-  const uint32_t sy = (nby + 7) >> 3, sz = (nbz + 7) >> 3;
-  const uint32_t xl = super_brick_xlog(bricks_along(g.xe - g.xb, g.bl[0]), g.xl_cap);
+#else
+  return magic ? (uint32_t)(((uint64_t)n * magic) >> 32) : n / d;
+#endif
+}
+__host__ __device__ __forceinline__ void brick_coords_in(uint32_t xl, uint32_t sy, uint32_t sz, uint32_t sy_magic, uint32_t sz_magic, uint32_t brick,
+                                                uint32_t* bx, uint32_t* by, uint32_t* bz) {
   const uint32_t sb = brick >> (6 + xl), in = brick & ((64u << xl) - 1u);
-  const uint32_t t = div_magic(sb, sz, g.sz_magic), sbz = sb - t * sz;
-  const uint32_t sbx = div_magic(t, sy, g.sy_magic), sby = t - sbx * sy;
+  const uint32_t t = div_magic(sb, sz, sz_magic), sbz = sb - t * sz;
+  const uint32_t sbx = div_magic(t, sy, sy_magic), sby = t - sbx * sy;
   *bx = (sbx << xl) + (in >> 6);
   *by = sby * 8 + ((in >> 3) & 7u);
   *bz = sbz * 8 + (in & 7u);
 }
+__device__ __forceinline__ void brick_coords(const GridParams& g, uint32_t brick, uint32_t* bx, uint32_t* by, uint32_t* bz) {
+  const uint32_t nby = bricks_along(g.n[1], g.bl[1]), nbz = bricks_along(g.n[2], g.bl[2]);
+  const uint32_t xl = super_brick_xlog(bricks_along(g.xe - g.xb, g.bl[0]), g.xl_cap);
+  brick_coords_in(xl, super_bricks_along(nby), super_bricks_along(nbz), g.sy_magic, g.sz_magic, brick, bx, by, bz);
+}
+__device__ __forceinline__ GridBrick grid_lane_voxel_of(const GridParams& g, uint32_t layers, uint32_t bx, uint32_t by, uint32_t bz, int lane);
 __device__ __forceinline__ GridBrick grid_lane_voxel(const GridParams& g, uint32_t brick, int lane) {
   uint32_t bx, by, bz;
   brick_coords(g, brick, &bx, &by, &bz);
+  return grid_lane_voxel_of(g, g.xe - g.xb, bx, by, bz, lane);
+}
+__device__ __forceinline__ GridBrick grid_lane_voxel(const GridParams& g, const PacketConsts& k, uint32_t brick, int lane) {
+  uint32_t bx, by, bz;
+  brick_coords_in(k.xl, k.sy, k.sz, k.sy_magic, k.sz_magic, brick, &bx, &by, &bz);
+  return grid_lane_voxel_of(g, k.layers, bx, by, bz, lane);
+}
+__device__ __forceinline__ GridBrick grid_lane_voxel_of(const GridParams& g, uint32_t layers, uint32_t bx, uint32_t by, uint32_t bz, int lane) {
   GridBrick v;
   const uint32_t lx = g.bl[0], ly = g.bl[1], lz = g.bl[2], l = (uint32_t)lane;
-  const uint32_t layers = g.xe - g.xb, xv = (bx << lx) + (l >> (ly + lz));
+  const uint32_t xv = (bx << lx) + (l >> (ly + lz));
   v.y = (by << ly) + ((l >> lz) & ((1u << ly) - 1u));
   v.z = (bz << lz) + (l & ((1u << lz) - 1u));
   v.in_range = xv < layers && v.y < g.n[1] && v.z < g.n[2];
```

Result: faster. 18000 Mvoxels/s, median of 6 (+1.6%).
